# hahnyuan/PTQ4ViT

Hardware: AMD Instinct MI355X
Metric: calibration throughput (wrapped modules calibrated per second), ViT-B/224 W8A8, 32 calibration images (higher is better)
Workload: dtype int8

## Files before the change

### include/ptq4vit_hip.h

```cpp
#ifndef PTQ4VIT_HIP_H
#define PTQ4VIT_HIP_H

#include <stddef.h>
#include <stdint.h>

#ifdef __cplusplus
extern "C" {
#endif

#define P4V_VERSION 140

enum p4v_metric {
    P4V_METRIC_L1_NORM = 0,
    P4V_METRIC_L2_NORM = 1,
    P4V_METRIC_LINEAR_WEIGHTED_L2 = 2,
    P4V_METRIC_SQUARE_WEIGHTED_L2 = 3,
    P4V_METRIC_HESSIAN = 4,
    P4V_METRIC_COSINE = 5
};

enum p4v_status {
    P4V_OK = 0,
    P4V_ERR_INVALID = -1,
    P4V_ERR_UNSUPPORTED = -2,
    P4V_ERR_WORKSPACE = -3,
    P4V_ERR_HIP = -4
};

int p4v_version(void);
const char* p4v_last_error(void);

typedef struct p4v_linear_desc {
    int32_t batch;
    int32_t tokens;
    int32_t in_features;
    int32_t out_features;
    int32_t n_V, n_H, n_a;
    int32_t w_bit, a_bit;
    int32_t metric;
    int32_t eq_n;
    int32_t search_round;
    int32_t twin_postgelu;
    int32_t init_layerwise;
    int32_t has_bias;
    int32_t reserved;
} p4v_linear_desc;

size_t p4v_linear_workspace_bytes(const p4v_linear_desc* desc);

int p4v_linear_calibrate(const p4v_linear_desc* desc, const float* d_weight, const float* d_bias,
                         const float* d_x, const float* d_out, const float* d_grad, const float* d_mult,
                         float* d_w_interval, float* d_a_interval, float* d_scores, int32_t* d_best,
                         void* d_workspace, size_t workspace_bytes, void* stream);

typedef struct p4v_matmul_desc {
    int32_t batch, heads;
    int32_t M, K, N;
    int64_t a_stride[4];
    int64_t b_stride[4];
    int32_t A_bit, B_bit;
    int32_t metric;
    int32_t eq_n;
    int32_t search_round;
    int32_t sos;
    int32_t init_layerwise;
    int32_t reserved;
} p4v_matmul_desc;

size_t p4v_matmul_workspace_bytes(const p4v_matmul_desc* desc);

int p4v_matmul_calibrate(const p4v_matmul_desc* desc, const float* d_A, const float* d_B, const float* d_out,
                         const float* d_grad, const float* d_mult, float* d_A_interval, float* d_B_interval,
                         float* d_split, float* d_scores, int32_t* d_best, void* d_workspace,
                         size_t workspace_bytes, void* stream);

typedef struct p4v_conv_desc {
    int32_t batch, in_channels, height, width;
    int32_t out_channels, kernel_h, kernel_w;
    int32_t stride_h, stride_w, pad_h, pad_w, dil_h, dil_w;
    int32_t w_bit, a_bit;
    int32_t metric;
    int32_t eq_n;
    int32_t search_round;
    int32_t channelwise;
    int32_t init_layerwise;
    int32_t has_bias;
    int32_t reserved;
} p4v_conv_desc;

size_t p4v_conv_workspace_bytes(const p4v_conv_desc* desc);

int p4v_conv_calibrate(const p4v_conv_desc* desc, const float* d_weight, const float* d_bias, const float* d_x,
                       const float* d_out, const float* d_grad, const float* d_mult, float* d_w_interval,
                       float* d_a_interval, float* d_scores, int32_t* d_best, void* d_workspace,
                       size_t workspace_bytes, void* stream);

enum p4v_job_kind { P4V_JOB_LINEAR = 0, P4V_JOB_MATMUL = 1, P4V_JOB_CONV = 2 };
typedef struct p4v_group_job {
    int32_t kind;
    int32_t status;
    const void* desc;
    const float* in[5];
    const float* mult;
    float* out[3];
    void* workspace;
    size_t workspace_bytes;
} p4v_group_job;
int p4v_calibrate_group(p4v_group_job* jobs, int32_t n_jobs, void* stream, void* inputs_ready_event);

int p4v_launch_counters(int64_t* out4, int reset);


int p4v_amax_init_linear(const p4v_linear_desc* desc, const float* d_weight, const float* d_x, float* d_w_interval,
                         float* d_a_interval, void* d_workspace, size_t workspace_bytes, void* stream);

int p4v_linear_search_w(const p4v_linear_desc* desc, const float* d_weight, const float* d_bias, const float* d_x,
                        const float* d_out, const float* d_grad, const float* d_w_cands, float* d_w_interval,
                        const float* d_a_interval, float* d_scores, int32_t* d_best, void* d_workspace,
                        size_t workspace_bytes, void* stream);

int p4v_linear_search_a(const p4v_linear_desc* desc, const float* d_weight, const float* d_bias, const float* d_x,
                        const float* d_out, const float* d_grad, const float* d_a_cands, const float* d_w_interval,
                        float* d_a_interval, float* d_scores, int32_t* d_best, void* d_workspace, size_t workspace_bytes,
                        void* stream);

int p4v_amax_init_matmul(const p4v_matmul_desc* desc, const float* d_A, const float* d_B, float* d_A_interval,
                         float* d_B_interval, void* d_workspace, size_t workspace_bytes, void* stream);

int p4v_matmul_search_A(const p4v_matmul_desc* desc, const float* d_A, const float* d_B, const float* d_out,
                        const float* d_grad, const float* d_A_cands, float* d_A_interval, const float* d_B_interval,
                        float* d_scores, int32_t* d_best, void* d_workspace, size_t workspace_bytes, void* stream);

int p4v_sos_search_split(const p4v_matmul_desc* desc, const float* d_A, const float* d_B, const float* d_out,
                         const float* d_grad, float* d_split, float* d_A_interval, float* d_scores, int32_t* d_best,
                         void* d_workspace, size_t workspace_bytes, void* stream);

int p4v_matmul_search_B(const p4v_matmul_desc* desc, const float* d_A, const float* d_B, const float* d_out,
                        const float* d_grad, const float* d_B_cands, const float* d_A_interval, const float* d_split,
                        float* d_B_interval, float* d_scores, int32_t* d_best, void* d_workspace, size_t workspace_bytes,
                        void* stream);

int p4v_amax_init_conv(const p4v_conv_desc* desc, const float* d_weight, const float* d_x, float* d_w_interval,
                       float* d_a_interval, void* d_workspace, size_t workspace_bytes, void* stream);

int p4v_conv_search_w_channelwise(const p4v_conv_desc* desc, const float* d_weight, const float* d_bias, const float* d_x,
                                  const float* d_out, const float* d_grad, const float* d_w_cands, float* d_w_interval,
                                  const float* d_a_interval, float* d_scores, int32_t* d_best, void* d_workspace,
                                  size_t workspace_bytes, void* stream);

int p4v_conv_search_w_layerwise(const p4v_conv_desc* desc, const float* d_weight, const float* d_bias, const float* d_x,
                                const float* d_out, const float* d_grad, const float* d_w_cands, float* d_w_interval,
                                const float* d_a_interval, float* d_scores, int32_t* d_best, void* d_workspace,
                                size_t workspace_bytes, void* stream);

int p4v_conv_search_a(const p4v_conv_desc* desc, const float* d_weight, const float* d_bias, const float* d_x,
                      const float* d_out, const float* d_grad, const float* d_a_cands, const float* d_w_interval,
                      float* d_a_interval, float* d_scores, int32_t* d_best, void* d_workspace, size_t workspace_bytes,
                      void* stream);

int p4v_score_argmax_gather(const float* d_scores, int32_t eq_n, int32_t n_blocks, const float* d_cands,
                            float* d_interval, int32_t* d_best, void* stream);


int p4v_quantize_i8(const float* d_x, int64_t rows, int64_t cols, int64_t cols_padded, const float* d_scales,
                    int64_t rows_per_scale, int32_t lo, int32_t hi, int8_t* d_q, void* stream);

enum p4v_plane_mode { P4V_PLANE_SYM = 1, P4V_PLANE_SOS_HI = 2, P4V_PLANE_SOS_LO = 3, P4V_PLANE_TWIN = 4 };
typedef struct p4v_plane_desc {
    int64_t rows, cols, cols_padded;
    int64_t rows_per_scale;
    int32_t mode, lo, hi, qmax;
    float const_scale;
    int32_t reserved;
} p4v_plane_desc;
int p4v_pack_plane_i8(const p4v_plane_desc* desc, const float* d_x, const float* d_scales, int8_t* d_q, void* stream);

int p4v_fake_quant(const float* d_x, int64_t rows, int64_t cols, const float* d_scales, int64_t rows_per_scale,
                   int32_t lo, int32_t hi, float* d_y, void* stream);

enum p4v_export_mode { P4V_EXPORT_SYM_I8 = 0, P4V_EXPORT_SYM_F32 = 1, P4V_EXPORT_GELU_U8 = 2, P4V_EXPORT_SOS_U8 = 3 };
typedef struct p4v_export_desc {
    int32_t dims[4];
    int64_t src_stride[4];
    int64_t scale1_stride[4]; int32_t scale1_div[4];
    int64_t scale2_stride[4]; int32_t scale2_div[4];
    float scale2_const;
    int32_t mode, lo1, hi1, lo2, hi2, qmax;
    int32_t reserved;
} p4v_export_desc;
int p4v_export_quantize(const p4v_export_desc* desc, const float* d_src, const float* d_scale1, const float* d_scale2,
                        void* d_dst, void* stream);

int p4v_linear_quant_forward(const p4v_linear_desc* desc, const float* d_weight, const float* d_bias, const float* d_x,
                             const float* d_w_interval, const float* d_a_interval, float* d_out, void* d_workspace,
                             size_t workspace_bytes, void* stream);

int p4v_matmul_quant_forward(const p4v_matmul_desc* desc, const float* d_A, const float* d_B, const float* d_A_interval,
                             const float* d_B_interval, const float* d_split, float* d_out, void* d_workspace,
                             size_t workspace_bytes, void* stream);

int p4v_multi_copy(const int64_t* d_table, int32_t n, int64_t index, int64_t max_bytes, void* stream);

typedef struct p4v_kernel_stats {
    double sweep_i8_ms;
    int64_t sweep_i8_launches;
    double sweep_i8_macs;
    double sweep_f32_ms;
    int64_t sweep_f32_launches;
    double sweep_f32_macs;
    double sweep_i8_alg_macs;
    double sweep_f32_alg_macs;
    double sweep6_ms;
    int64_t sweep6_launches;
    double sweep6_macs;
    double sweep6_alg_macs;
    int64_t memo_hits;
    int64_t memo_misses;
    double sweep7_ms;
    int64_t sweep7_launches;
    double sweep7_macs;
    double sweep7_alg_macs;
    double sweep7_twin_ms;
    int64_t sweep7_twin_launches;
    double event_overhead_ms;
} p4v_kernel_stats;

typedef struct p4v_launch_record {
    int32_t kind;
    int32_t stage;
    int32_t grid_x, grid_z;
    double ms;
    double ops;
    double alg_ops;
    double alg_bytes;
} p4v_launch_record;
int p4v_stats_launches(p4v_launch_record* out, int64_t capacity, int64_t* count);

int p4v_stats_enable(int enable);
int p4v_stats_reset(void);
int p4v_stats_get(p4v_kernel_stats* out);

int p4v_prune_counters(int64_t* out4, int reset);


#ifdef __cplusplus
}
#endif
#endif
```

### include/ptq4vit_hip_debug.h

```cpp
#ifndef PTQ4VIT_HIP_DEBUG_H
#define PTQ4VIT_HIP_DEBUG_H

#include <stdint.h>

#ifdef __cplusplus
extern "C" {
#endif

int p4v_debug_set_variant(int variant, int force_generic);
int p4v_debug_set_tuning(int key, int value);
int p4v_debug_topk_rows(const float* d_mass, int segs, int n, int k, int32_t* d_idx, void* stream);
int p4v_debug_pack_dual(const float* d_x, long rows, long cols, long cols_padded, int sos, int lo, int hi, int qmax,
                        const float* d_scale, float const_scale, int8_t* d_q1, int8_t* d_q2, void* stream);
int p4v_debug_pack_cands(const float* d_x, long rows, long cols, long rows_padded, long cols_padded, int layout, int lo, int hi,
                         const float* d_scales, int n_cands, const int* d_crange, const unsigned char* d_done, int live_max,
                         int general, int8_t* d_q, void* stream);
int p4v_debug_prep_epi6(const float* d_o, const float* d_wt, const float* d_bias, long o_ss, long o_ts, int sr, int tr,
                        int bias_on_t, int wt_mode, int transposed, float* d_e, void* stream);

#ifdef __cplusplus
}
#endif
#endif
```

### ptq4vit_amd/_lib.py

```python
import ctypes as C
import os

_HERE = os.path.dirname(os.path.abspath(__file__))
LIB_PATH = os.environ.get("P4V_LIB") or os.path.join(_HERE, "csrc", "libptq4vit_hip.so")

METRICS = {
    "L1_norm": 0,
    "L2_norm": 1,
    "linear_weighted_L2_norm": 2,
    "square_weighted_L2_norm": 3,
    "hessian": 4,
    "cosine": 5,
}


class LinearDesc(C.Structure):
    _fields_ = [(n, C.c_int32) for n in (
        "batch", "tokens", "in_features", "out_features", "n_V", "n_H", "n_a", "w_bit", "a_bit", "metric",
        "eq_n", "search_round", "twin_postgelu", "init_layerwise", "has_bias", "reserved")]


class MatMulDesc(C.Structure):
    _fields_ = ([(n, C.c_int32) for n in ("batch", "heads", "M", "K", "N")] + [("_pad0", C.c_int32)] +
                [("a_stride", C.c_int64 * 4), ("b_stride", C.c_int64 * 4)] +
                [(n, C.c_int32) for n in ("A_bit", "B_bit", "metric", "eq_n", "search_round", "sos",
                                          "init_layerwise", "reserved")])


class ConvDesc(C.Structure):
    _fields_ = [(n, C.c_int32) for n in (
        "batch", "in_channels", "height", "width", "out_channels", "kernel_h", "kernel_w", "stride_h", "stride_w",
        "pad_h", "pad_w", "dil_h", "dil_w", "w_bit", "a_bit", "metric", "eq_n", "search_round", "channelwise",
        "init_layerwise", "has_bias", "reserved")]


class KernelStats(C.Structure):
    _fields_ = [("sweep_i8_ms", C.c_double), ("sweep_i8_launches", C.c_int64), ("sweep_i8_macs", C.c_double),
                ("sweep_f32_ms", C.c_double), ("sweep_f32_launches", C.c_int64), ("sweep_f32_macs", C.c_double),
                ("sweep_i8_alg_macs", C.c_double), ("sweep_f32_alg_macs", C.c_double),
                ("sweep6_ms", C.c_double), ("sweep6_launches", C.c_int64), ("sweep6_macs", C.c_double), ("sweep6_alg_macs", C.c_double),
                ("memo_hits", C.c_int64), ("memo_misses", C.c_int64),
                ("sweep7_ms", C.c_double), ("sweep7_launches", C.c_int64), ("sweep7_macs", C.c_double), ("sweep7_alg_macs", C.c_double),
                ("sweep7_twin_ms", C.c_double), ("sweep7_twin_launches", C.c_int64), ("event_overhead_ms", C.c_double)]


class LaunchRecord(C.Structure):
    _fields_ = [("kind", C.c_int32), ("stage", C.c_int32), ("grid_x", C.c_int32), ("grid_z", C.c_int32),
                ("ms", C.c_double), ("ops", C.c_double), ("alg_ops", C.c_double), ("alg_bytes", C.c_double)]


LAUNCH_KINDS = {0: "k_sweep<int8>", 1: "k_sweep<float>", 2: "k_sweep6", 3: "k_sweep7", 4: "k_sweep7 (twin)", 5: "k_sweep4/5", 6: "k_sweep9",
                7: "k_sweep8", 8: "k_sweep2g", 9: "k_sweep2", 11: "k_sos_split", 12: "k_bound", 13: "k_slice_b", 14: "k_slice_a"}
LAUNCH_STAGES = {0: "full", 1: "A", 2: "B1", 3: "B2", 4: "A2"}


class PlaneDesc(C.Structure):
    _fields_ = [("rows", C.c_int64), ("cols", C.c_int64), ("cols_padded", C.c_int64), ("rows_per_scale", C.c_int64),
                ("mode", C.c_int32), ("lo", C.c_int32), ("hi", C.c_int32), ("qmax", C.c_int32),
                ("const_scale", C.c_float), ("reserved", C.c_int32)]


class ExportDesc(C.Structure):
    _fields_ = [("dims", C.c_int32 * 4), ("src_stride", C.c_int64 * 4),
                ("scale1_stride", C.c_int64 * 4), ("scale1_div", C.c_int32 * 4),
                ("scale2_stride", C.c_int64 * 4), ("scale2_div", C.c_int32 * 4),
                ("scale2_const", C.c_float),
                ("mode", C.c_int32), ("lo1", C.c_int32), ("hi1", C.c_int32), ("lo2", C.c_int32), ("hi2", C.c_int32),
                ("qmax", C.c_int32), ("reserved", C.c_int32)]


class GroupJob(C.Structure):
    _fields_ = [("kind", C.c_int32), ("status", C.c_int32), ("desc", C.c_void_p), ("inp", C.c_void_p * 5), ("mult", C.c_void_p),
                ("out", C.c_void_p * 3), ("workspace", C.c_void_p), ("workspace_bytes", C.c_size_t)]


JOB_LINEAR, JOB_MATMUL, JOB_CONV = 0, 1, 2
PLANE_SYM, PLANE_SOS_HI, PLANE_SOS_LO, PLANE_TWIN = 1, 2, 3, 4
EXPORT_SYM_I8, EXPORT_SYM_F32, EXPORT_GELU_U8, EXPORT_SOS_U8 = 0, 1, 2, 3


EXPORTS = [
    "p4v_version", "p4v_last_error",
    "p4v_linear_workspace_bytes", "p4v_linear_calibrate",
    "p4v_matmul_workspace_bytes", "p4v_matmul_calibrate",
    "p4v_conv_workspace_bytes", "p4v_conv_calibrate",
    "p4v_calibrate_group", "p4v_launch_counters",
    "p4v_linear_quant_forward", "p4v_matmul_quant_forward",
    "p4v_amax_init_linear", "p4v_linear_search_w", "p4v_linear_search_a",
    "p4v_amax_init_matmul", "p4v_matmul_search_A", "p4v_sos_search_split", "p4v_matmul_search_B",
    "p4v_amax_init_conv", "p4v_conv_search_w_channelwise", "p4v_conv_search_w_layerwise", "p4v_conv_search_a",
    "p4v_score_argmax_gather",
    "p4v_quantize_i8", "p4v_pack_plane_i8", "p4v_fake_quant", "p4v_export_quantize", "p4v_multi_copy",
    "p4v_stats_enable", "p4v_stats_reset", "p4v_stats_get", "p4v_stats_launches", "p4v_prune_counters",
    "p4v_debug_set_variant", "p4v_debug_set_tuning", "p4v_debug_topk_rows", "p4v_debug_pack_dual", "p4v_debug_prep_epi6",
    "p4v_debug_pack_cands",
]

_lib = None


def load():
    global _lib
    if _lib is not None:
        return _lib
    if not os.path.exists(LIB_PATH):
        raise RuntimeError(
            f"ptq4vit_amd: HIP extension {LIB_PATH} is missing -- build it with "
            "`python -c 'import __graft_entry__ as g; g.build()'` (hipcc --offload-arch=gfx950). "
            "There is no CPU fallback for the calibration path.")
    import torch
    lib = C.CDLL(LIB_PATH)
    vp, fp, ip = C.c_void_p, C.c_void_p, C.c_void_p
    lib.p4v_version.restype = C.c_int
    lib.p4v_last_error.restype = C.c_char_p
    lib.p4v_linear_workspace_bytes.restype = C.c_size_t
    lib.p4v_linear_workspace_bytes.argtypes = [C.POINTER(LinearDesc)]
    lib.p4v_linear_calibrate.restype = C.c_int
    lib.p4v_linear_calibrate.argtypes = [C.POINTER(LinearDesc), fp, fp, fp, fp, fp, fp, fp, fp, fp, ip, vp, C.c_size_t, vp]
    lib.p4v_matmul_workspace_bytes.restype = C.c_size_t
    lib.p4v_matmul_workspace_bytes.argtypes = [C.POINTER(MatMulDesc)]
    lib.p4v_matmul_calibrate.restype = C.c_int
    lib.p4v_matmul_calibrate.argtypes = [C.POINTER(MatMulDesc), fp, fp, fp, fp, fp, fp, fp, fp, fp, ip, vp, C.c_size_t, vp]
    lib.p4v_conv_workspace_bytes.restype = C.c_size_t
    lib.p4v_conv_workspace_bytes.argtypes = [C.POINTER(ConvDesc)]
    lib.p4v_conv_calibrate.restype = C.c_int
    lib.p4v_conv_calibrate.argtypes = [C.POINTER(ConvDesc), fp, fp, fp, fp, fp, fp, fp, fp, fp, ip, vp, C.c_size_t, vp]
    lib.p4v_linear_quant_forward.restype = C.c_int
    lib.p4v_linear_quant_forward.argtypes = [C.POINTER(LinearDesc), fp, fp, fp, fp, fp, fp, vp, C.c_size_t, vp]
    lib.p4v_matmul_quant_forward.restype = C.c_int
    lib.p4v_matmul_quant_forward.argtypes = [C.POINTER(MatMulDesc), fp, fp, fp, fp, fp, fp, vp, C.c_size_t, vp]
    LD, MD, CD = C.POINTER(LinearDesc), C.POINTER(MatMulDesc), C.POINTER(ConvDesc)
    tail = [vp, C.c_size_t, vp]
    for name, args in (
            ("p4v_amax_init_linear", [LD] + [fp] * 4),
            ("p4v_linear_search_w", [LD] + [fp] * 9 + [ip]),
            ("p4v_linear_search_a", [LD] + [fp] * 9 + [ip]),
            ("p4v_amax_init_matmul", [MD] + [fp] * 4),
            ("p4v_matmul_search_A", [MD] + [fp] * 8 + [ip]),
            ("p4v_sos_search_split", [MD] + [fp] * 7 + [ip]),
            ("p4v_matmul_search_B", [MD] + [fp] * 9 + [ip]),
            ("p4v_amax_init_conv", [CD] + [fp] * 4),
            ("p4v_conv_search_w_channelwise", [CD] + [fp] * 9 + [ip]),
            ("p4v_conv_search_w_layerwise", [CD] + [fp] * 9 + [ip]),
            ("p4v_conv_search_a", [CD] + [fp] * 9 + [ip])):
        fn = getattr(lib, name)
        fn.restype = C.c_int
        fn.argtypes = args + tail
    lib.p4v_score_argmax_gather.restype = C.c_int
    lib.p4v_score_argmax_gather.argtypes = [fp, C.c_int32, C.c_int32, fp, fp, ip, vp]
    lib.p4v_quantize_i8.restype = C.c_int
    lib.p4v_quantize_i8.argtypes = [fp, C.c_int64, C.c_int64, C.c_int64, fp, C.c_int64, C.c_int32, C.c_int32, vp, vp]
    lib.p4v_fake_quant.restype = C.c_int
    lib.p4v_fake_quant.argtypes = [fp, C.c_int64, C.c_int64, fp, C.c_int64, C.c_int32, C.c_int32, fp, vp]
    lib.p4v_pack_plane_i8.restype = C.c_int
    lib.p4v_pack_plane_i8.argtypes = [C.POINTER(PlaneDesc), fp, fp, vp, vp]
    lib.p4v_export_quantize.restype = C.c_int
    lib.p4v_export_quantize.argtypes = [C.POINTER(ExportDesc), fp, fp, fp, vp, vp]
    lib.p4v_multi_copy.restype = C.c_int
    lib.p4v_multi_copy.argtypes = [vp, C.c_int32, C.c_int64, C.c_int64, vp]
    lib.p4v_debug_topk_rows.restype = C.c_int
    lib.p4v_debug_topk_rows.argtypes = [vp, C.c_int, C.c_int, C.c_int, vp, vp]
    lib.p4v_debug_pack_dual.restype = C.c_int
    lib.p4v_debug_pack_dual.argtypes = [fp, C.c_long, C.c_long, C.c_long, C.c_int, C.c_int, C.c_int, C.c_int, fp, C.c_float, vp, vp, vp]
    lib.p4v_debug_pack_cands.restype = C.c_int
    lib.p4v_debug_pack_cands.argtypes = [fp, C.c_long, C.c_long, C.c_long, C.c_long, C.c_int, C.c_int, C.c_int, fp, C.c_int, vp, vp,
                                         C.c_int, C.c_int, vp, vp]
    lib.p4v_debug_prep_epi6.restype = C.c_int
    lib.p4v_debug_prep_epi6.argtypes = [fp, fp, fp, C.c_long, C.c_long, C.c_int, C.c_int, C.c_int, C.c_int, C.c_int, fp, vp]
    lib.p4v_debug_set_variant.restype = C.c_int
    lib.p4v_debug_set_variant.argtypes = [C.c_int, C.c_int]
    lib.p4v_debug_set_tuning.restype = C.c_int
    lib.p4v_debug_set_tuning.argtypes = [C.c_int, C.c_int]
    lib.p4v_stats_enable.restype = C.c_int
    lib.p4v_stats_enable.argtypes = [C.c_int]
    lib.p4v_stats_reset.restype = C.c_int
    lib.p4v_stats_get.restype = C.c_int
    lib.p4v_stats_get.argtypes = [C.POINTER(KernelStats)]
    lib.p4v_stats_launches.restype = C.c_int
    lib.p4v_stats_launches.argtypes = [C.POINTER(LaunchRecord), C.c_int64, C.POINTER(C.c_int64)]
    lib.p4v_prune_counters.restype = C.c_int
    lib.p4v_prune_counters.argtypes = [C.POINTER(C.c_int64), C.c_int]
    lib.p4v_launch_counters.restype = C.c_int
    lib.p4v_launch_counters.argtypes = [C.POINTER(C.c_int64), C.c_int]
    lib.p4v_calibrate_group.restype = C.c_int
    lib.p4v_calibrate_group.argtypes = [C.POINTER(GroupJob), C.c_int32, vp, vp]
    _lib = lib
    return lib


def check(rc, what):
    if rc != 0:
        msg = load().p4v_last_error().decode("utf-8", "replace")
        if rc == -2:
            raise NotImplementedError(f"{what}: {msg}")
        raise RuntimeError(f"{what} failed (code {rc}): {msg}")


def source_hash():
    import hashlib
    root = os.path.dirname(os.path.abspath(__file__))
    h = hashlib.sha256()
    for rel in ("csrc/p4v_kernels.h", "csrc/p4v_api.hip", "../include/ptq4vit_hip.h"):
        with open(os.path.join(root, rel), "rb") as f:
            h.update(f.read())
    return h.hexdigest()[:16]
```

### ptq4vit_amd/csrc/p4v_api.hip

```cpp
#include <hip/hip_runtime.h>

#include <algorithm>
#include <atomic>
#include <climits>
#include <cstdarg>
#include <cstdio>
#include <condition_variable>
#include <cstring>
#include <deque>
#include <functional>
#include <thread>
#include <mutex>
#include <string>
#include <unordered_map>
#include <type_traits>
#include <vector>

#include "../../include/ptq4vit_hip.h"
#include "../../include/ptq4vit_hip_debug.h"
#include "p4v_kernels.h"

using namespace p4v;

namespace {
// ... 24 lines not shown
inline long rup(long x, long m) { return (x + m - 1) / m * m; }
inline int cdiv(long a, long b) { return (int)((a + b - 1) / b); }

struct Arena {
    char* base;
    size_t cap, off, peak;
    size_t top;
    bool dry;
    Arena(void* b, size_t c) : base((char*)b), cap(c & ~(size_t)255), off(0), peak(0), top(0), dry(b == nullptr) {}
    template <typename T> T* get(size_t n) {
        off = (size_t)rup((long)off, 256);
        T* p = dry ? nullptr : (T*)(base + off);
        off += n * sizeof(T);
        if (off + top > peak) peak = off + top;
        return p;
    }
    char* get_top(size_t bytes) {
        top += (size_t)rup((long)bytes, 256);
        if (off + top > peak) peak = off + top;
        return (dry || top > cap) ? nullptr : base + cap - top;
    }
    bool ok() const { return dry || off + top <= cap; }
};

struct StatRec { hipEvent_t a, b; int kind; double macs, alg; int stage, gx, gz; double ms, bytes; };
thread_local double g_alg_bytes = 0;
thread_local double g_alg_macs_cand = 0;
thread_local double g_exec_frac = 1.0;
thread_local bool g_stat_on = false;
thread_local std::vector<StatRec> g_stat_recs;
thread_local std::vector<StatRec> g_stat_done;
thread_local int g_stage = 0;
thread_local p4v_kernel_stats g_stats = {};
thread_local long g_memo_hits = 0, g_memo_misses = 0;
std::atomic<long long> g_prune_cnt[4];
constexpr int VARIANT_KEPT = 1 | 2 | 4 | 2048 | 32768 | 65536 | 131072 | 524288 | 1048576 | 2097152 | 4194304 | 8388608 | 134217728;
std::atomic<int> g_variant_word{0};
#define g_variant (g_variant_word.load(std::memory_order_relaxed) & 0x3fffffff)
#define g_force_v1 ((g_variant_word.load(std::memory_order_relaxed) >> 30) & 1)
std::atomic<int> g_tune[16];
enum { TUNE_CG6 = 0, TUNE_CG2 = 1, TUNE_CG2G = 2, TUNE_CG7 = 3, TUNE_PRINT = 4, TUNE_ORDER7 = 5, TUNE_P6 = 6, TUNE_PLANE_GIB = 7, TUNE_EPI6W = 8,
       TUNE_LOOSE_PCT = 9, TUNE_SLICE_DIV = 10, TUNE_SLICE_SMALL = 11, TUNE_B1_PATH = 12, TUNE_TIER2 = 13, TUNE_TIER2_DIV = 14, TUNE_LOOSE_ROWS = 15 };
inline bool tune_b1_removed(int v) { return v == 1 || v == 2 || v == 3 || v == 5 || v == 6 || v == 8 || v == 10 || v == 12; }
inline int tune(int k) { return g_tune[k].load(std::memory_order_relaxed); }

struct Group;
struct Ctx {
    hipStream_t st;
    Arena ws;
    bool dry;
    Group* grp = nullptr;
    int slot = 0;
    int par = 1;
};

struct StatInfo { int kind; double macs, alg; int stage, gx, gz; double bytes; };
struct QOp;
struct KernelDesc {
    hipError_t (*one)(const QOp&, hipStream_t);
    hipError_t (*many)(const QOp* const*, int, hipStream_t);
    int cap;
};
constexpr int QOP_PARAM_BYTES = 480;
struct QOp {
    enum Type : int { KERNEL, FILL, D2H, H2D, COPY2D, WAIT };
    int type = KERNEL;
    const KernelDesc* kd = nullptr;
    dim3 grid, block;
    unsigned lds = 0;
    alignas(16) char params[QOP_PARAM_BYTES];
    void* dst = nullptr; const void* src = nullptr; size_t bytes = 0; int value = 0;
    size_t dpitch = 0, spitch = 0, width = 0, height = 0;
    std::vector<char> payload;
    bool timed = false;
    bool heavy = false;
    StatInfo si{};
};
inline hipError_t lds_attr(const void* fn, unsigned lds, std::atomic<bool>& done) {
    if (lds <= 48 * 1024 || done.load(std::memory_order_acquire)) return hipSuccess;
    const hipError_t e = hipFuncSetAttribute(fn, hipFuncAttributeMaxDynamicSharedMemorySize, 160 * 1024);
    if (e == hipSuccess) done.store(true, std::memory_order_release);
    return e;
}
template <typename P, void (*K1)(P), void (*KG)(GroupArgs<P>)> struct Kern {
    static_assert(sizeof(P) <= QOP_PARAM_BYTES, "kernel parameter block larger than a queued operation holds");
    static hipError_t one(const QOp& op, hipStream_t st) {
        static std::atomic<bool> attr{false};
        if (hipError_t e = lds_attr((const void*)K1, op.lds, attr); e != hipSuccess) return e;
        P p;
        std::memcpy(&p, op.params, sizeof(P));
        void* args[] = {&p};
        return hipLaunchKernel((const void*)K1, op.grid, op.block, args, op.lds, st);
    }
    static hipError_t many(const QOp* const* ops, int n, hipStream_t st) {
        static std::atomic<bool> attr{false};
        GroupArgs<P> a;
        unsigned off = 0, lds = 0;
        a.n = n;
        for (int m = 0; m < n; ++m) {
            const QOp& op = *ops[m];
            a.off[m] = off; a.gx[m] = op.grid.x; a.gy[m] = op.grid.y; a.gz[m] = op.grid.z;
            std::memcpy(&a.p[m], op.params, sizeof(P));
            off += (unsigned)rup((long)op.grid.x * op.grid.y * op.grid.z, 8);
            lds = std::max(lds, op.lds);
        }
        a.off[n] = off;
        if (hipError_t e = lds_attr((const void*)KG, lds, attr); e != hipSuccess) return e;
// ... 1059 lines not shown
        const bool cosp = ps.cos6 || ps.cos7;
        const int cos6_FS = !cosp ? 0 : ps.cos_ZV == 1 ? cos6_slabs : ps.sb_div / cos_slab;
        FinishCosParams fp{part, p_cs, cosp ? (long)cos6_FS * cos6_Sp * 3 : p_zs, cosp ? cos6_Sp : Np, cosp ? cos6_FS : MT,
                           ps.cos_ZB, ps.cos_ZV, cosp ? ps.Mrows : ps.Ncols, ps.eq_n,
                           ps.cos_j_mode, std::max(1, ps.cos_j_div), ps.nj, ps.norm, scores};
        CHK(launch_finish_cos(c, fp));
    }
    if (!ps.no_select) {
        SelectParams sl{scores, ps.eq_n, ps.nj, ps.cands, ps.cand_cs, ps.cand_js, ps.cand_off, ps.interval, ps.out_js,
                        ps.out_off, ps.aux_out, ps.aux_div, ps.scores_out, ps.scores_out_ld, ps.best_out};
        CHK(launch_select(c, sl));
    }
    c.ws.off = mark;
    return 0;
}

struct SliceGeo {
    bool lin; int segs, seg_rows, k , Ncols, K;
    const float* O; const float* G; int wt_mode; long o_ms;
    const float* row_src; long s_r, s_k; int zdiv; long s_z2, s_z;
    bool conv; PackParams conv_pk;
    int k_cap;
};
int slice_alloc(Ctx& c, SliceCache* sc, const SliceGeo& g, bool keep, bool bump) {
    if (sc->assigned) {
        if (sc->k != g.k_cap) return fail(P4V_ERR_INVALID, "slice cache reused with another geometry");
        return 0;
    }
    if (!keep && !bump) return 0;
    const long zrows = (long)g.segs * g.seg_rows, out_elems = (long)g.segs * g.k_cap * g.Ncols, row_elems = (long)g.segs * g.k_cap * g.K;
    if (keep) {
        sc->idx = reinterpret_cast<int*>(c.ws.get_top((size_t)g.segs * g.k_cap * sizeof(int)));
        sc->mass = reinterpret_cast<float*>(c.ws.get_top((size_t)zrows * sizeof(float)));
        sc->Os = reinterpret_cast<float*>(c.ws.get_top((size_t)out_elems * sizeof(float)));
        sc->Gs = reinterpret_cast<float*>(c.ws.get_top((size_t)out_elems * sizeof(float)));
        sc->Rs = reinterpret_cast<float*>(c.ws.get_top((size_t)row_elems * sizeof(float)));
        sc->frac = reinterpret_cast<float*>(c.ws.get_top(256));
        sc->assigned = true;
    } else {
        sc->idx = c.ws.get<int>((size_t)g.segs * g.k_cap);
        sc->mass = c.ws.get<float>((size_t)zrows);
        sc->Os = c.ws.get<float>((size_t)out_elems);
        sc->Gs = c.ws.get<float>((size_t)out_elems);
        sc->Rs = c.ws.get<float>((size_t)row_elems);
    }
    sc->k = g.k_cap;
    return 0;
}
int slice_fill(Ctx& c, SliceCache* sc, const SliceGeo& g, bool host_sync_ok) {
    const long zrows = (long)g.segs * g.seg_rows;
    const void* wsrc = g.G ? (const void*)g.G : (const void*)g.O;
    const bool new_idx = sc->idx_src != wsrc || sc->idx_wt != g.wt_mode || (g.wt_mode != 1 && sc->o_src != g.O);
    if (new_idx) {
        CHK(enqueue(c, KERN(RowMassParams, k_row_mass), dim3((unsigned)cdiv(zrows, 4)), dim3(256), 0, RowMassParams{g.G ? g.G : g.O, g.O, zrows, (long)g.Ncols, g.wt_mode, sc->mass}));
        CHK(enqueue(c, KERN(TopkParams, k_topk_rows), dim3(g.segs), dim3(1024), 0, TopkParams{sc->mass, g.seg_rows, g.k, sc->idx}));
        sc->idx_src = wsrc; sc->idx_wt = g.wt_mode;
        sc->o_src = sc->g_src = sc->r_src = nullptr;
        if (sc->frac && host_sync_ok && !(g_variant & 8388608)) {
            float f = 1.0f;
            int* hm = host_mirror(c);
            CHK(enqueue(c, KERN(MassFracParams, k_mass_fraction), dim3(1), dim3(1024), 0,
                        MassFracParams{sc->mass, zrows, sc->idx, g.segs, g.seg_rows, g.k, sc->frac, hm ? reinterpret_cast<float*>(hm + 4) : nullptr}));
            if (!hm) CHK(q_d2h(c, &f, sc->frac, sizeof f));
            CHK(q_sync(c));
            if (hm) f = *reinterpret_cast<volatile float*>(hm + 4);
            if (tune(TUNE_PRINT) > 0) fprintf(stderr, "[p4v] slice holds %.4f of the metric weight (%d x %d of %d rows)\n", f, g.segs, g.k, g.seg_rows);
            sc->frac_host = f;
            if (g.k < g.k_cap && !(f >= 0.97f)) {
                SliceGeo g2 = g;
                g2.k = g.k_cap;
                sc->idx_src = nullptr;
                return slice_fill(c, sc, g2, host_sync_ok);
            }
            const bool big_pass = zrows >= (tune(TUNE_LOOSE_ROWS) > 0 ? (long)tune(TUNE_LOOSE_ROWS) : 65536L);
            if (!(f >= (tune(TUNE_LOOSE_PCT) > 0 ? 0.01f * tune(TUNE_LOOSE_PCT) : big_pass ? 0.05f : 0.5f))) { sc->loose = true; return 0; }
        }
        sc->k_eff = g.k;
    }
    const int rows = g.segs * g.k;
    int gather_rc = 0;
    auto gather = [&](const float* src, long s0, long s3, int d3, float* dst, int seg, int zdiv, long sz2, long sz) {
        GatherParams gp{src, s0, 0, 0, s3, 1, 1, d3, sc->idx, rows, dst, seg, zdiv, sz2, sz};
        const long total = (long)rows * d3;
        if (const int r_ = enqueue(c, KERN(GatherParams, k_gather), dim3((unsigned)std::min<long>(cdiv(total, 256), 256L * 16)), dim3(256), 0, gp)) gather_rc = r_;
    };
    const int seg = g.lin ? 0 : g.k;
    const long o_seg = (long)g.seg_rows * g.Ncols;
    if (sc->o_src != g.O) { gather(g.O, g.o_ms, 1, g.Ncols, sc->Os, seg, 1, o_seg, 0); sc->o_src = g.O; }
    if (g.G && sc->g_src != g.G) { gather(g.G, g.o_ms, 1, g.Ncols, sc->Gs, seg, 1, o_seg, 0); sc->g_src = g.G; }
    if (sc->r_src != g.row_src) {
        if (g.conv) {
            const long total = (long)rows * g.K;
            CHK(enqueue(c, KERN(GatherIm2colParams, k_gather_im2col), dim3((unsigned)std::min<long>(cdiv(total, 256), 256L * 16)), dim3(256), 0, GatherIm2colParams{g.conv_pk, sc->idx, rows, sc->Rs}));
        } else if (g.lin) gather(g.row_src, g.s_r, 1, g.K, sc->Rs, 0, 1, 0, 0);
        else gather(g.row_src, g.s_r, g.s_k, g.K, sc->Rs, g.k, g.zdiv, g.s_z2, g.s_z);
        sc->r_src = g.row_src;
        sc->aplane.valid = false;
    }
    return gather_rc;
}

bool prune_ok(const Pass& ps) {
    if (!ps.prunable || !(ps.i8 || ps.prunable_f32) || ps.epi == EPI_COS || ps.store_out || ps.scores_out || ps.best_out || ps.crange || ps.no_select) return false;
    if ((g_variant & 4194304) || ps.eq_n < 32 || ps.nj < 1 || ps.nj > 4096) return false;
    return true;
}
int launch_pass_select(Ctx& c, const Pass& ps, const float* scores) {
    SelectParams sl{scores, ps.eq_n, ps.nj, ps.cands, ps.cand_cs, ps.cand_js, ps.cand_off, ps.interval, ps.out_js,
                    ps.out_off, ps.aux_out, ps.aux_div, ps.scores_out, ps.scores_out_ld, ps.best_out};
    return launch_select(c, sl);
}

#define PRUNE_COUNT(i) do { if (!c.dry) g_prune_cnt[i].fetch_add(1, std::memory_order_relaxed); } while (0)
constexpr int PRUNE_FP32_CHAIN = 128 + 6;
inline float prune_margin() { return std::max(1e-4f, 4.0f * 2.0f * (float)PRUNE_FP32_CHAIN * 5.9604645e-8f); }
// ... 477 lines not shown
    bool full() const { return mask == ST_ALL; }
    bool searches() const { return (mask & (ST_S1 | ST_S2)) != 0; }
};

PackParams pack2d(const float* src, long rows, long cols, long ld) {
    PackParams p{};
    p.src = src; p.s_z = 0; p.s_r = ld; p.s_k = 1; p.Z = 1; p.R = (int)rows; p.K = (int)cols;
    p.mode = PACK_SYM; p.nblk_r = 1; p.nblk_k = 1;
    return p;
}

int linear_impl(const p4v_linear_desc* d, const float* W, const float* bias, const float* X, const float* O,
                const float* G, const float* mult, float* w_iv, float* a_iv, float* scores_out, int32_t* best_out,
                Ctx& c, float* fwd_out = nullptr, const Stage& sg = Stage{}) {
    const int M = d->batch * d->tokens, K = d->in_features, N = d->out_features;
    const int nV = d->n_V, nH = d->n_H, nA = d->n_a;
    if (M <= 0 || K <= 0 || N <= 0 || nV <= 0 || nH <= 0 || nA <= 0 || d->eq_n <= 0)
        return fail(P4V_ERR_INVALID, "linear: non-positive dimension");
    if (N % nV || K % nH || K % nA) return fail(P4V_ERR_UNSUPPORTED, "linear: n_V/n_H/n_a must divide the layer (reference ignores remainders, linear.py:118)");
    if (d->w_bit > 8 || d->a_bit > 8 || d->w_bit < 2 || d->a_bit < 2) return fail(P4V_ERR_UNSUPPORTED, "linear: bit widths 2..8 supported");
    const int crb_rows = N / nV, crb_cols = K / nH, crb_acts = K / nA;
    const int wq = 1 << (d->w_bit - 1), aq = 1 << (d->a_bit - 1);
    const float a_neg = (float)(0.16997124254703522 / aq);
    int epi, wt_mode;
    metric_epi(d->metric, &epi, &wt_mode);
    const bool cosm = epi == EPI_COS;
    if (wt_mode == 1 && !G && !fwd_out && sg.searches()) return fail(P4V_ERR_INVALID, "linear: hessian metric needs raw_grad (linear.py:418)");
    const bool general = (nH > 1 || nA > 1 || (d->reserved & 1) || (cosm && d->twin_postgelu && !fwd_out));
    const bool i8 = !general;
    const bool twin = d->twin_postgelu && i8;
    if (cosm && !fwd_out && (nH > 1 || nA > 1)) return fail(P4V_ERR_UNSUPPORTED, "linear: cosine with n_H>1 / n_a>1 is not implemented on the GPU");
    const int ncand = d->eq_n + 1;

    cvt_bias(c);
    unsigned* enc_w = c.ws.get<unsigned>((size_t)nV * nH);
    unsigned* enc_a = c.ws.get<unsigned>((size_t)nA);
    float* w_cands_ws = c.ws.get<float>((size_t)ncand * nV * nH);
    float* a_cands_ws = c.ws.get<float>((size_t)ncand * nA);
    const float* w_cands = (sg.mask & ST_INIT) ? w_cands_ws : sg.cands1;
    const float* a_cands = (sg.mask & ST_INIT) ? a_cands_ws : sg.cands2;
    float* Ufold = twin ? c.ws.get<float>((size_t)M * N) : nullptr;
    float* w_mix = c.ws.get<float>((size_t)ncand * nV * nH);
    float* a_mix = c.ws.get<float>((size_t)ncand * nA);
    if (!c.ws.ok()) return fail(P4V_ERR_WORKSPACE, "workspace too small");
    if (!fwd_out && (sg.mask & ST_INIT)) {
        const long stw[4] = {0, 0, K, 1};
        CHK(launch_absmax(c, W, stw, 1, 1, N, K, nV, nH, crb_rows, crb_cols, 0, enc_w));
        CHK(launch_interval(c, enc_w, nV * nH, (float)(wq - 0.5), d->init_layerwise, w_iv));
        if (sg.searches()) CHK(launch_cands(c, mult, w_iv, ncand, nV * nH, w_cands_ws));
    }
    auto init_activation_side = [&]() -> int {
        if (!fwd_out && (sg.mask & ST_INIT)) {
            const long stw[4] = {0, 0, K, 1};
            CHK(launch_absmax(c, X, stw, 1, 1, M, K, 1, nA, M, crb_acts, d->twin_postgelu ? 1 : 0, enc_a));
            CHK(launch_interval(c, enc_a, nA, (float)(aq - 0.5), d->init_layerwise, a_iv));
            if (sg.searches()) CHK(launch_cands(c, mult, a_iv, ncand, nA, a_cands_ws));
        }
        return 0;
    };
    if (fwd_out || !sg.full()) {
        CHK(q_wait_inputs(c));
        CHK(init_activation_side());
    }
    if (!fwd_out && !sg.searches()) return 0;

    auto x_operand = [&](bool expanded, const float* scales, int sc_cs) {
        Operand op{};
        op.present = true; op.expanded = expanded;
        op.pk = pack2d(X, M, K, K);
        op.pk.scales = scales; op.pk.sc_cs = sc_cs;
        op.pk.lo = -aq; op.pk.hi = aq - 1;
        if (nA > 1) { op.pk.blk_mode = 1; op.pk.blk_div = INT_MAX; op.pk.nblk_r = 1; op.pk.nblk_k = nA; op.pk.blk_div2 = crb_acts; }
        if (d->twin_postgelu) {
            if (i8) { op.pk.lo = 0; }
            else { op.pk.mode = PACK_TWIN_SIM; op.pk.lo = -aq; op.pk.neg_scale = a_neg; }
        }
        return op;
    };
    auto xneg_operand = [&]() {
        Operand op{};
        op.present = true; op.expanded = false;
        op.pk = pack2d(X, M, K, K);
        op.pk.scales = nullptr; op.pk.neg_scale = a_neg; op.pk.lo = -aq; op.pk.hi = 0;
        return op;
    };
    auto w_operand = [&](bool expanded, const float* scales, int sc_cs, bool by_vblock) {
        Operand op{};
        op.present = true; op.expanded = expanded;
        if (by_vblock) {
            op.pk = pack2d(W, crb_rows, K, K);
            op.pk.s_z = (long)crb_rows * K;
            op.pk.blk_mode = 2; op.pk.blk_div = nV;
            if (nH > 1) return op;
        } else {
            op.pk = pack2d(W, N, K, K);
            op.pk.blk_mode = 1; op.pk.blk_div = crb_rows; op.pk.nblk_r = nV; op.pk.nblk_k = nH;
            op.pk.blk_div2 = nH > 1 ? crb_cols : 0;
        }
        op.pk.scales = scales; op.pk.sc_cs = sc_cs;
        op.pk.lo = -wq; op.pk.hi = wq - 1;
        return op;
    };

    if (fwd_out) {
        Pass fp{};
        fp.i8 = i8; fp.twin = twin; fp.epi = EPI_FWD; fp.wt_mode = 0; fp.eq_n = 1; fp.K = K;
        fp.Z = 1; fp.Mrows = M; fp.Ncols = N;
        fp.row = x_operand(false, a_iv, 0);
// ... 154 lines not shown
                    slice2.o_src = nullptr;
                }
                if (cos6 || cos7) cos6_pass(ps, 0);
            } else {
                ps.Z = nV; ps.Mrows = crb_rows; ps.Ncols = M;
                ps.row = w_operand(false, w_iv, 0, true);
                ps.col = x_operand(true, ac, nA);
                ps.col_zs_shared = 1;
                ps.use_s1 = i8; ps.s_cs = nV; ps.sb_mode = 2; ps.sb_div = nV;
                ps.s1 = ScaleParams{a_cands, 1, 0, 0.f, w_iv, 0, 1, 0.f, 0, 0, nullptr};
                ps.bias = bias; ps.bias_axis = 1; ps.bias_zs = crb_rows;
                ps.O = O; ps.o_zs = crb_rows; ps.o_ms = 1; ps.o_ns = N; ps.o_inner = INT_MAX;
                ps.cos_ZB = 1; ps.cos_ZV = nV; ps.cos_j_mode = 0;
                ps.norm = 1.0 / (double)d->tokens;
            }
            CHK(run_pass_pruned(c, ps));
        }
        if (memo_a_on && !skip_a) { CHK(read_dev(c, a_iv, nA, val)); memo_a.entries.push_back({key, val}); g_memo_misses++; host_a = val; host_a_ok = true; }
        else if (!skip_a) host_a_ok = false;
    }
    return 0;
}

int matmul_impl(const p4v_matmul_desc* d, const float* A, const float* B, const float* O, const float* G,
                const float* mult, float* A_iv, float* B_iv, float* split, float* scores_out, int32_t* best_out, Ctx& c,
                float* fwd_out = nullptr, const Stage& sg = Stage{}) {
    const int H = d->heads, Z = d->batch * d->heads, M = d->M, K = d->K, N = d->N;
    if (Z <= 0 || M <= 0 || K <= 0 || N <= 0 || d->eq_n <= 0) return fail(P4V_ERR_INVALID, "matmul: non-positive dimension");
    if (d->A_bit > 8 || d->B_bit > 8) return fail(P4V_ERR_UNSUPPORTED, "matmul: bit widths <= 8 supported");
    const int Aq = 1 << (d->A_bit - 1), Bq = 1 << (d->B_bit - 1);
    int epi, wt_mode;
    metric_epi(d->metric, &epi, &wt_mode);
    const bool cosm = epi == EPI_COS;
    if (wt_mode == 1 && !G && !fwd_out && sg.searches()) return fail(P4V_ERR_INVALID, "matmul: hessian metric needs raw_grad");
    if (d->sos && !split) return fail(P4V_ERR_INVALID, "matmul: sos needs d_split");
    cvt_bias(c);
    CHK(q_wait_inputs(c));
    const int ncand = d->eq_n + 1;
    const int NSPLIT = 20;

    unsigned* enc_A = c.ws.get<unsigned>(H);
    unsigned* enc_B = c.ws.get<unsigned>(H);
    float* A_cands_ws = c.ws.get<float>((size_t)ncand * H);
    float* B_cands_ws = c.ws.get<float>((size_t)ncand * H);
    const float* A_cands = (sg.mask & ST_INIT) ? A_cands_ws : sg.cands1;
    const float* B_cands = (sg.mask & ST_INIT) ? B_cands_ws : sg.cands2;
    float* split_cands = c.ws.get<float>(NSPLIT);
    float* A_headwise = c.ws.get<float>(H);
    if (!c.ws.ok()) return fail(P4V_ERR_WORKSPACE, "workspace too small");
    if (!fwd_out && (sg.mask & ST_INIT)) {
        const long sa[4] = {d->a_stride[0], d->a_stride[1], d->a_stride[2], d->a_stride[3]};
        const long sb[4] = {d->b_stride[0], d->b_stride[1], d->b_stride[2], d->b_stride[3]};
        float* a_dst = d->sos ? A_headwise : A_iv;
        CHK(launch_absmax(c, A, sa, d->batch, H, M, K, 1, 1, M, K, 0, enc_A));
        CHK(launch_interval(c, enc_A, H, (float)(Aq - 0.5), d->init_layerwise, a_dst));
        CHK(launch_absmax(c, B, sb, d->batch, H, K, N, 1, 1, K, N, 0, enc_B));
        CHK(launch_interval(c, enc_B, H, (float)(Bq - 0.5), d->init_layerwise, B_iv));
        if (sg.searches()) {
            if (!d->sos) CHK(launch_cands(c, mult, A_iv, ncand, H, A_cands_ws));
            CHK(launch_cands(c, mult, B_iv, ncand, H, B_cands_ws));
        }
    }
    if (!fwd_out && !sg.searches()) return 0;
    if (!fwd_out && (sg.mask & ST_S1)) {
        if (d->sos && !c.dry) {
            float sc[NSPLIT];
            for (int i = 0; i < NSPLIT; ++i) sc[i] = (float)std::ldexp(1.0, -i);
            CHK(q_h2d(c, split_cands, sc, sizeof sc));
            if (!c.grp) CHK(q_sync(c));
        }
    }
    auto A_operand = [&](bool expanded, const float* scales, int sc_cs, int mode) {
        Operand op{};
        op.present = true; op.expanded = expanded;
        op.pk = PackParams{};
        op.pk.src = A; op.pk.s_z = d->a_stride[1]; op.pk.s_r = d->a_stride[2]; op.pk.s_k = d->a_stride[3];
        op.pk.s_z2 = d->a_stride[0]; op.pk.zdiv = H;
        op.pk.Z = Z; op.pk.R = M; op.pk.K = K; op.pk.nblk_r = 1; op.pk.nblk_k = 1;
        op.pk.mode = mode; op.pk.scales = scales; op.pk.sc_cs = sc_cs;
        op.pk.blk_mode = (mode == PACK_SYM) ? 2 : 0; op.pk.blk_div = H;
        op.pk.lo = -Aq; op.pk.hi = Aq - 1; op.pk.qm1 = (float)(Aq - 1);
        return op;
    };
    auto B_operand = [&](bool expanded, const float* scales, int sc_cs, int mode) {
        Operand op{};
        op.present = true; op.expanded = expanded;
        op.pk = PackParams{};
        op.pk.src = B; op.pk.s_z = d->b_stride[1]; op.pk.s_r = d->b_stride[3]; op.pk.s_k = d->b_stride[2];
        op.pk.s_z2 = d->b_stride[0]; op.pk.zdiv = H;
        op.pk.Z = Z; op.pk.R = N; op.pk.K = K; op.pk.nblk_r = 1; op.pk.nblk_k = 1;
        op.pk.mode = mode; op.pk.scales = scales; op.pk.sc_cs = sc_cs;
        op.pk.blk_mode = (mode == PACK_SYM) ? 2 : 0; op.pk.blk_div = H;
        op.pk.lo = -Bq; op.pk.hi = Bq - 1;
        return op;
    };
    auto common = [&](Pass& ps) {
        ps.Z = Z; ps.K = K;
        ps.O = O; ps.G = G; ps.wt_mode = wt_mode; ps.epi = epi;
        ps.o_inner = INT_MAX;
        if (!cosm) { ps.Mrows = M; ps.Ncols = N; ps.o_zs = (long)M * N; ps.o_ms = N; ps.o_ns = 1; }
        else { ps.Mrows = N; ps.Ncols = M; ps.o_zs = (long)M * N; ps.o_ms = 1; ps.o_ns = N; ps.G = nullptr;
               ps.cos_ZB = Z; ps.cos_ZV = 1; }
    };

    if (fwd_out) {
        Pass fp{};
        fp.Z = Z; fp.K = K; fp.Mrows = M; fp.Ncols = N;
        fp.i8 = true; fp.twin = d->sos; fp.epi = EPI_FWD; fp.wt_mode = 0; fp.eq_n = 1;
        fp.row = d->sos ? A_operand(false, split, 0, PACK_SOS_HI) : A_operand(false, A_iv, 0, PACK_SYM);
        if (d->sos) fp.row2 = A_operand(false, split, 0, PACK_SOS_LO);
// ... 104 lines not shown
                ps.s1 = ScaleParams{nullptr, 0, 0, 1.0f / (float)(Aq - 1), B_cands, H, 1, 0.f, 0, 0, nullptr};
                ps.s2 = ScaleParams{A_iv, 0, 0, 0.f, B_cands, H, 1, 0.f, 0, 0, nullptr};
            }
            ps.j_mode = 2; ps.j_div = H; ps.nj = H; ps.cos_j_mode = 2; ps.cos_j_div = H;
            ps.norm = cosm ? 1.0 / (double)M : 1.0 / ((double)M * N);
            ps.cands = B_cands; ps.cand_cs = H; ps.cand_js = 1; ps.interval = B_iv; ps.out_js = 1;
            ps.cache = keep_planes ? &plane_B : nullptr;
            ps.scores_out = so_B; ps.scores_out_ld = H;
            ps.best_out = bo_B;
            ps.prunable = !cosm && ps.i8 && !(d->reserved & 8); ps.scache = &slice; ps.host_sync_ok = memo_on;
            CHK(run_pass_pruned(c, ps));
            if (memo_on) { CHK(read_dev(c, B_iv, H, val)); memo_B.entries.push_back({key, val}); g_memo_misses++; }
        }
    }
    return 0;
}

int conv_impl(const p4v_conv_desc* d, const float* W, const float* bias, const float* X, const float* O, const float* G,
              const float* mult, float* w_iv, float* a_iv, float* scores_out, int32_t* best_out, Ctx& c,
              const Stage& sg = Stage{}) {
    const int b = d->batch, ic = d->in_channels, H = d->height, Wd = d->width, oc = d->out_channels;
    const int kh = d->kernel_h, kw = d->kernel_w;
    const int fh = (H + 2 * d->pad_h - d->dil_h * (kh - 1) - 1) / d->stride_h + 1;
    const int fw = (Wd + 2 * d->pad_w - d->dil_w * (kw - 1) - 1) / d->stride_w + 1;
    if (b <= 0 || ic <= 0 || oc <= 0 || fh <= 0 || fw <= 0 || d->eq_n <= 0) return fail(P4V_ERR_INVALID, "conv: bad geometry");
    if (d->w_bit > 8) return fail(P4V_ERR_UNSUPPORTED, "conv: w_bit <= 8 supported");
    const int L = fh * fw, K = ic * kh * kw, M = b * L;
    const int wq = 1 << (d->w_bit - 1);
    const bool aquant = d->a_bit < 32;
    const int aq = aquant ? (1 << (d->a_bit - 1)) : 0;
    if (aquant && !d->channelwise) return fail(P4V_ERR_UNSUPPORTED, "conv: the layer-wise class cannot search activations (reference conv.py:420 raises IndexError); use a_bit=32");
    cvt_bias(c);
    CHK(q_wait_inputs(c));
    int epi, wt_mode;
    metric_epi(d->metric, &epi, &wt_mode);
    const bool cosm = epi == EPI_COS;
    if (wt_mode == 1 && !G && sg.searches()) return fail(P4V_ERR_INVALID, "conv: hessian metric needs raw_grad");
    if (cosm && aquant) return fail(P4V_ERR_UNSUPPORTED, "conv: cosine does not support the activation search (reference conv.py:505-506)");
    const int nw = d->channelwise ? oc : 1;
    const int ncand = d->eq_n + 1;

    unsigned* enc_w = c.ws.get<unsigned>(nw);
    unsigned* enc_a = c.ws.get<unsigned>(1);
    float* w_cands_ws = c.ws.get<float>((size_t)ncand * nw);
    float* a_cands_ws = c.ws.get<float>(ncand);
    const float* w_cands = (sg.mask & ST_INIT) ? w_cands_ws : sg.cands1;
    const float* a_cands = (sg.mask & ST_INIT) ? a_cands_ws : sg.cands2;
    if (!c.ws.ok()) return fail(P4V_ERR_WORKSPACE, "workspace too small");
    if (sg.mask & ST_INIT) {
        const long stw[4] = {0, 0, K, 1};
        CHK(launch_absmax(c, W, stw, 1, 1, oc, K, nw, 1, d->channelwise ? 1 : oc, K, 0, enc_w));
        CHK(launch_interval(c, enc_w, nw, (float)(wq - 0.5), d->init_layerwise, w_iv));
        const long stx[4] = {0, 0, (long)ic * H * Wd, 1};
        CHK(launch_absmax(c, X, stx, 1, 1, b, ic * H * Wd, 1, 1, b, ic * H * Wd, 0, enc_a));
        CHK(launch_interval(c, enc_a, 1, aquant ? (float)(aq - 0.5) : (float)(std::ldexp(1.0, d->a_bit - 1) - 0.5), 0, a_iv));
        if (sg.searches()) {
            CHK(launch_cands(c, mult, w_iv, ncand, nw, w_cands_ws));
            CHK(launch_cands(c, mult, a_iv, ncand, 1, a_cands_ws));
        }
    }
    if (!sg.searches()) return 0;
    const bool prunable = !cosm && sg.full() && !scores_out && !best_out && !(d->reserved & 8) && d->eq_n >= 32;
    float* Ot = prunable ? c.ws.get<float>((size_t)M * oc) : nullptr;
    float* Gt = (prunable && G) ? c.ws.get<float>((size_t)M * oc) : nullptr;
    if (!c.ws.ok()) return fail(P4V_ERR_WORKSPACE, "workspace too small");
    if (prunable && !c.dry) {
        const dim3 grid(cdiv(L, 32), cdiv(oc, 32), b);
        CHK(enqueue(c, KERN(NchwRowsParams, k_nchw_to_rows), grid, dim3(256), 0, NchwRowsParams{O, oc, L, Ot}));
        if (G) CHK(enqueue(c, KERN(NchwRowsParams, k_nchw_to_rows), grid, dim3(256), 0, NchwRowsParams{G, oc, L, Gt}));
    }
    auto x_operand = [&](bool expanded, const float* scales, int sc_cs, bool per_image) {
        Operand op{};
        op.present = true; op.expanded = expanded;
        op.pk = PackParams{};
        op.pk.src = X; op.pk.conv = 1; op.pk.ic = ic; op.pk.H = H; op.pk.W = Wd; op.pk.kh = kh; op.pk.kw = kw;
        op.pk.sh = d->stride_h; op.pk.sw = d->stride_w; op.pk.ph = d->pad_h; op.pk.pw = d->pad_w; op.pk.dh = d->dil_h; op.pk.dw = d->dil_w;
        op.pk.fw = fw; op.pk.L = L;
        op.pk.Z = per_image ? b : 1; op.pk.s_z = per_image ? (long)ic * H * Wd : 0;
        op.pk.R = per_image ? L : M; op.pk.K = K; op.pk.nblk_r = 1; op.pk.nblk_k = 1;
        op.pk.mode = aquant ? PACK_SYM : PACK_RAW; op.pk.scales = aquant ? scales : nullptr; op.pk.sc_cs = sc_cs;
        op.pk.lo = -aq; op.pk.hi = aq - 1;
        return op;
    };
    auto w_operand = [&](bool expanded, const float* scales, int sc_cs) {
        Operand op{};
        op.present = true; op.expanded = expanded;
        op.pk = pack2d(W, oc, K, K);
        op.pk.scales = scales; op.pk.sc_cs = sc_cs;
        op.pk.blk_mode = d->channelwise ? 1 : 0; op.pk.blk_div = 1; op.pk.nblk_r = nw; op.pk.nblk_k = 1;
        op.pk.lo = -wq; op.pk.hi = wq - 1;
        return op;
    };
    auto setup = [&](Pass& ps, bool w_search) {
        ps.i8 = false; ps.twin = false; ps.epi = epi; ps.wt_mode = wt_mode; ps.eq_n = d->eq_n; ps.K = K;
        ps.use_s1 = false; ps.s_cs = 1; ps.sb_mode = 0;
        ps.O = O; ps.G = G; ps.bias = bias;
        Operand xo = x_operand(!w_search, w_search ? a_iv : a_cands, w_search ? 0 : 1, cosm && d->channelwise);
        Operand wo = w_operand(w_search, w_search ? w_cands : w_iv, w_search ? nw : 0);
        if (!cosm) {
            ps.Z = 1; ps.Mrows = M; ps.Ncols = oc; ps.row = xo; ps.col = wo;
            ps.o_inner = L; ps.o_bs = (long)oc * L; ps.o_ms = 1; ps.o_ns = L; ps.bias_axis = 0;
            if (prunable) { ps.O = Ot; ps.G = G ? Gt : nullptr; ps.o_inner = INT_MAX; ps.o_bs = 0; ps.o_ms = oc; ps.o_ns = 1; }
        } else if (d->channelwise) {
            ps.Z = b; ps.Mrows = L; ps.Ncols = oc; ps.row = xo; ps.col = wo; ps.col_zs_shared = 1;
            ps.o_zs = (long)oc * L; ps.o_inner = INT_MAX; ps.o_ms = 1; ps.o_ns = L; ps.bias_axis = 0; ps.G = nullptr;
            ps.cos_ZB = b; ps.cos_ZV = 1;
        } else {
            ps.Z = 1; ps.Mrows = oc; ps.Ncols = M; ps.row = wo; ps.col = xo;
// ... 157 lines not shown
    return linear_impl(desc, d_weight, desc->has_bias ? d_bias : nullptr, d_x, nullptr, nullptr, nullptr,
                       const_cast<float*>(d_w_interval), const_cast<float*>(d_a_interval), nullptr, nullptr, c, d_out);
}

int p4v_matmul_quant_forward(const p4v_matmul_desc* desc, const float* d_A, const float* d_B, const float* d_A_interval,
                             const float* d_B_interval, const float* d_split, float* d_out, void* d_workspace,
                             size_t workspace_bytes, void* stream) {
    if (!desc || !d_A || !d_B || !d_A_interval || !d_B_interval || !d_out || !d_workspace)
        return fail(P4V_ERR_INVALID, "p4v_matmul_quant_forward: null pointer");
    if (desc->sos && !d_split) return fail(P4V_ERR_INVALID, "p4v_matmul_quant_forward: sos needs d_split");
    Ctx c{(hipStream_t)stream, Arena(d_workspace, workspace_bytes), false};
    return matmul_impl(desc, d_A, d_B, nullptr, nullptr, nullptr, const_cast<float*>(d_A_interval),
                       const_cast<float*>(d_B_interval), const_cast<float*>(d_split), nullptr, nullptr, c, d_out);
}

size_t p4v_matmul_workspace_bytes(const p4v_matmul_desc* desc) {
    if (!desc) return 0;
    Ctx c{nullptr, Arena(nullptr, 0), true};
    float dummy = 0;
    float* fwd = (desc->reserved & 4) ? (float*)16 : nullptr;
    if (matmul_impl(desc, nullptr, nullptr, nullptr, (const float*)1, nullptr, nullptr, nullptr, &dummy, nullptr, nullptr, c, fwd) != 0) return 0;
    return c.ws.peak + 4096;
}

int p4v_matmul_calibrate(const p4v_matmul_desc* desc, const float* d_A, const float* d_B, const float* d_out,
                         const float* d_grad, const float* d_mult, float* d_A_interval, float* d_B_interval, float* d_split,
                         float* d_scores, int32_t* d_best, void* d_workspace, size_t workspace_bytes, void* stream) {
    if (!desc || !d_A || !d_B || !d_out || !d_mult || !d_A_interval || !d_B_interval || !d_workspace)
        return fail(P4V_ERR_INVALID, "matmul: null pointer");
    Ctx c{(hipStream_t)stream, Arena(d_workspace, workspace_bytes), false};
    return matmul_impl(desc, d_A, d_B, d_out, d_grad, d_mult, d_A_interval, d_B_interval, d_split, d_scores, d_best, c);
}

size_t p4v_conv_workspace_bytes(const p4v_conv_desc* desc) {
    if (!desc) return 0;
    Ctx c{nullptr, Arena(nullptr, 0), true};
    if (conv_impl(desc, nullptr, nullptr, nullptr, nullptr, (const float*)1, nullptr, nullptr, nullptr, nullptr, nullptr, c) != 0) return 0;
    return c.ws.peak + 4096;
}

int p4v_conv_calibrate(const p4v_conv_desc* desc, const float* d_weight, const float* d_bias, const float* d_x,
                       const float* d_out, const float* d_grad, const float* d_mult, float* d_w_interval, float* d_a_interval,
                       float* d_scores, int32_t* d_best, void* d_workspace, size_t workspace_bytes, void* stream) {
    if (!desc || !d_weight || !d_x || !d_out || !d_mult || !d_w_interval || !d_a_interval || !d_workspace)
        return fail(P4V_ERR_INVALID, "conv: null pointer");
    if (desc->has_bias && !d_bias) return fail(P4V_ERR_INVALID, "conv: has_bias set but d_bias is NULL");
    Ctx c{(hipStream_t)stream, Arena(d_workspace, workspace_bytes), false};
    return conv_impl(desc, d_weight, desc->has_bias ? d_bias : nullptr, d_x, d_out, d_grad, d_mult, d_w_interval, d_a_interval,
                     d_scores, d_best, c);
}


int p4v_calibrate_group(p4v_group_job* jobs, int32_t n_jobs, void* stream, void* inputs_ready_event) {
    if (n_jobs < 0 || (n_jobs > 0 && !jobs)) return fail(P4V_ERR_INVALID, "p4v_calibrate_group: bad job list");
    if (n_jobs == 0) return 0;
    for (int i = 0; i < n_jobs; ++i) {
        jobs[i].status = 0;
        if (!jobs[i].desc || group_desc_bytes(jobs[i].kind) == 0) return fail(P4V_ERR_INVALID, "p4v_calibrate_group: member %d has no descriptor / an unknown kind", i);
    }
    int dev = 0;
    HIPCHK(hipGetDevice(&dev));
    cvt_probe((hipStream_t)stream);
    Group g;
    g.st = (hipStream_t)stream; g.n = n_jobs;
    g.q.resize(n_jobs); g.state.assign(n_jobs, 0); g.mirrors.resize(n_jobs);
    for (int i = 0; i < n_jobs; ++i) g.mirrors[i] = group_mirror(g.st, dev, i);
    g.stat_on = g_stat_on;
    g.stat_recs = g_stat_on ? &g_stat_recs : nullptr;
    g.inputs_ready = (hipEvent_t)inputs_ready_event;
    g_launch_cnt[3].fetch_add(1, std::memory_order_relaxed);
    std::vector<std::string> errs(n_jobs);
    std::atomic<long> memo_hits{0}, memo_misses{0};
    std::mutex dmu;
    std::condition_variable dcv;
    int left = n_jobs;
    for (int i = 0; i < n_jobs; ++i) {
        int par = 0;
        for (int k = 0; k < n_jobs; ++k)
            par += jobs[k].kind == jobs[i].kind && std::memcmp(jobs[k].desc, jobs[i].desc, group_desc_bytes(jobs[i].kind)) == 0;
        worker_pool().run([&, i, par] {
            (void)hipSetDevice(dev);
            g_stat_on = g.stat_on; g_stage = 0; g_exec_frac = 1.0; g_memo_hits = 0; g_memo_misses = 0; g_err.clear();
            Ctx c{g.st, Arena(jobs[i].workspace, jobs[i].workspace_bytes), false, &g, i, par};
            const int r = run_group_member(jobs[i], c);
            jobs[i].status = r;
            if (r) errs[i] = g_err;
            memo_hits += g_memo_hits; memo_misses += g_memo_misses;
            g_stat_on = false;
            g.finish(i);
            std::lock_guard<std::mutex> lk(dmu);
            if (--left == 0) dcv.notify_all();
        });
    }
    {
        std::unique_lock<std::mutex> lk(dmu);
        dcv.wait(lk, [&] { return left == 0; });
    }
    g_memo_hits += memo_hits.load(); g_memo_misses += memo_misses.load();
    if (tune(TUNE_PRINT) > 0) fprintf(stderr, "[p4v] group of %d: %ld launches asked for, %ld issued in %ld rounds\n", n_jobs, g.n_ops, g.n_launches, g.n_rounds);
    if (g.status) { g_err = g.err; return g.status; }
    for (int i = 0; i < n_jobs; ++i)
        if (jobs[i].status) { g_err = errs[i]; return jobs[i].status; }
    return 0;
}

int p4v_launch_counters(int64_t* out4, int reset) {
    if (out4) for (int i = 0; i < 4; ++i) out4[i] = (int64_t)g_launch_cnt[i].load(std::memory_order_relaxed);
    if (reset) for (int i = 0; i < 4; ++i) g_launch_cnt[i].store(0, std::memory_order_relaxed);
    return 0;
}

int p4v_amax_init_linear(const p4v_linear_desc* desc, const float* d_weight, const float* d_x, float* d_w_interval,
                         float* d_a_interval, void* d_workspace, size_t workspace_bytes, void* stream) {
    if (!desc || !d_weight || !d_x || !d_w_interval || !d_a_interval || !d_workspace)
        return fail(P4V_ERR_INVALID, "p4v_amax_init_linear: null pointer");
    Ctx c{(hipStream_t)stream, Arena(d_workspace, workspace_bytes), false};
    return linear_impl(desc, d_weight, nullptr, d_x, nullptr, nullptr, nullptr, d_w_interval, d_a_interval, nullptr, nullptr, c,
                       nullptr, Stage{ST_INIT, nullptr, nullptr});
}

int p4v_linear_search_w(const p4v_linear_desc* desc, const float* d_weight, const float* d_bias, const float* d_x,
                        const float* d_out, const float* d_grad, const float* d_w_cands, float* d_w_interval,
                        const float* d_a_interval, float* d_scores, int32_t* d_best, void* d_workspace,
                        size_t workspace_bytes, void* stream) {
    if (!desc || !d_weight || !d_x || !d_out || !d_w_cands || !d_w_interval || !d_a_interval || !d_workspace)
        return fail(P4V_ERR_INVALID, "p4v_linear_search_w: null pointer");
    if (desc->has_bias && !d_bias) return fail(P4V_ERR_INVALID, "p4v_linear_search_w: has_bias set but d_bias is NULL");
    Ctx c{(hipStream_t)stream, Arena(d_workspace, workspace_bytes), false};
    return linear_impl(desc, d_weight, desc->has_bias ? d_bias : nullptr, d_x, d_out, d_grad, nullptr, d_w_interval,
                       const_cast<float*>(d_a_interval), d_scores, d_best, c, nullptr, Stage{ST_S1, d_w_cands, nullptr});
}

int p4v_linear_search_a(const p4v_linear_desc* desc, const float* d_weight, const float* d_bias, const float* d_x,
                        const float* d_out, const float* d_grad, const float* d_a_cands, const float* d_w_interval,
                        float* d_a_interval, float* d_scores, int32_t* d_best, void* d_workspace, size_t workspace_bytes,
                        void* stream) {
// ... 76 lines not shown
int p4v_conv_search_w_channelwise(const p4v_conv_desc* desc, const float* d_weight, const float* d_bias, const float* d_x,
                                  const float* d_out, const float* d_grad, const float* d_w_cands, float* d_w_interval,
                                  const float* d_a_interval, float* d_scores, int32_t* d_best, void* d_workspace,
                                  size_t workspace_bytes, void* stream) {
    return conv_search("p4v_conv_search_w_channelwise", 1, ST_S1, desc, d_weight, d_bias, d_x, d_out, d_grad, d_w_cands,
                       d_w_interval, const_cast<float*>(d_a_interval), d_scores, d_best, d_workspace, workspace_bytes, stream);
}

int p4v_conv_search_w_layerwise(const p4v_conv_desc* desc, const float* d_weight, const float* d_bias, const float* d_x,
                                const float* d_out, const float* d_grad, const float* d_w_cands, float* d_w_interval,
                                const float* d_a_interval, float* d_scores, int32_t* d_best, void* d_workspace,
                                size_t workspace_bytes, void* stream) {
    return conv_search("p4v_conv_search_w_layerwise", 0, ST_S1, desc, d_weight, d_bias, d_x, d_out, d_grad, d_w_cands,
                       d_w_interval, const_cast<float*>(d_a_interval), d_scores, d_best, d_workspace, workspace_bytes, stream);
}

int p4v_conv_search_a(const p4v_conv_desc* desc, const float* d_weight, const float* d_bias, const float* d_x,
                      const float* d_out, const float* d_grad, const float* d_a_cands, const float* d_w_interval,
                      float* d_a_interval, float* d_scores, int32_t* d_best, void* d_workspace, size_t workspace_bytes,
                      void* stream) {
    if (desc && desc->a_bit >= 32) return fail(P4V_ERR_INVALID, "p4v_conv_search_a: a_bit >= 32 leaves the input unquantised (conv.py:600)");
    return conv_search("p4v_conv_search_a", -1, ST_S2, desc, d_weight, d_bias, d_x, d_out, d_grad, d_a_cands,
                       const_cast<float*>(d_w_interval), d_a_interval, d_scores, d_best, d_workspace, workspace_bytes, stream);
}

int p4v_score_argmax_gather(const float* d_scores, int32_t eq_n, int32_t n_blocks, const float* d_cands, float* d_interval,
                            int32_t* d_best, void* stream) {
    if (!d_scores || !d_cands || !d_interval || eq_n <= 0 || n_blocks <= 0)
        return fail(P4V_ERR_INVALID, "p4v_score_argmax_gather: bad argument");
    Ctx c{(hipStream_t)stream, Arena(nullptr, 0), false};
    SelectParams sl{d_scores, eq_n, n_blocks, d_cands, n_blocks, 1, 0, d_interval, 1, 0, nullptr, 0.0f, nullptr, 0, d_best};
    return launch_select(c, sl);
}

int p4v_quantize_i8(const float* d_x, int64_t rows, int64_t cols, int64_t cols_padded, const float* d_scales,
                    int64_t rows_per_scale, int32_t lo, int32_t hi, int8_t* d_q, void* stream) {
    if (!d_x || !d_scales || !d_q || rows <= 0 || cols <= 0 || cols_padded % 64 || cols_padded < cols || rows_per_scale <= 0)
        return fail(P4V_ERR_INVALID, "quantize_i8: bad argument");
    Ctx c{(hipStream_t)stream, Arena(nullptr, 0), false};
    PackParams p = pack2d(d_x, rows, cols, cols);
    p.Rp = (int)rows; p.Kp = (int)cols_padded; p.dst = d_q; p.C = 1;
    p.scales = d_scales; p.sc_cs = 0; p.blk_mode = 1; p.blk_div = (int)rows_per_scale;
    p.nblk_r = cdiv(rows, rows_per_scale); p.nblk_k = 1; p.lo = lo; p.hi = hi;
    return launch_pack<int8_t>(c, p);
}

int p4v_fake_quant(const float* d_x, int64_t rows, int64_t cols, const float* d_scales, int64_t rows_per_scale,
                   int32_t lo, int32_t hi, float* d_y, void* stream) {
    if (!d_x || !d_scales || !d_y || rows <= 0 || cols <= 0 || rows_per_scale <= 0)
        return fail(P4V_ERR_INVALID, "fake_quant: bad argument");
    const long n = rows * cols;
    hipLaunchKernelGGL(k_fake_quant_rows, dim3((unsigned)std::min<long>(cdiv(n, 256), 65536)), dim3(256), 0,
                       (hipStream_t)stream, d_x, (long)rows, (long)cols, d_scales, (long)rows_per_scale, (float)lo, (float)hi, d_y);
    HIPCHK(hipGetLastError());
    return 0;
}

int p4v_multi_copy(const int64_t* d_table, int32_t n, int64_t index, int64_t max_bytes, void* stream) {
    if (!d_table || n <= 0 || index < 0 || max_bytes <= 0) return fail(P4V_ERR_INVALID, "p4v_multi_copy: bad argument");
    static_assert(sizeof(long) == sizeof(int64_t), "table entries are 64-bit");
    const unsigned gx = (unsigned)std::max<long>(1, std::min<long>(cdiv(max_bytes / 16, 256 * 8), 256));
    hipLaunchKernelGGL(k_multi_copy, dim3(gx, (unsigned)n), dim3(256), 0, (hipStream_t)stream, (const long*)d_table, (long)index);
    HIPCHK(hipGetLastError());
    return 0;
}

thread_local double g_evt_overhead_ms = 0.0;
int p4v_stats_enable(int enable) {
    g_stat_on = enable != 0;
    if (g_stat_on) {
        hipEvent_t a, b;
        HIPCHK(hipEventCreate(&a));
        HIPCHK(hipEventCreate(&b));
        double best = 1e9;
        for (int i = 0; i < 32; ++i) {
            HIPCHK(hipEventRecord(a, nullptr));
            HIPCHK(hipEventRecord(b, nullptr));
            HIPCHK(hipEventSynchronize(b));
            float ms = 0;
            HIPCHK(hipEventElapsedTime(&ms, a, b));
            best = std::min(best, (double)ms);
        }
        hipEventDestroy(a);
        hipEventDestroy(b);
        g_evt_overhead_ms = best < 1e8 ? best : 0.0;
    }
    return 0;
}

static int stats_drain() {
    for (auto& r : g_stat_recs) {
        HIPCHK(hipEventSynchronize(r.b));
        float ms = 0;
        HIPCHK(hipEventElapsedTime(&ms, r.a, r.b));
        ms = (float)std::max(0.0, (double)ms - g_evt_overhead_ms);
        if (r.kind == 0 || (r.kind >= 2 && r.kind <= 9) || (r.kind >= 12 && r.kind <= 14)) { g_stats.sweep_i8_ms += ms; g_stats.sweep_i8_launches++; g_stats.sweep_i8_macs += r.macs; g_stats.sweep_i8_alg_macs += r.alg; }
        if (r.kind == 2) { g_stats.sweep6_ms += ms; g_stats.sweep6_launches++; g_stats.sweep6_macs += r.macs; g_stats.sweep6_alg_macs += r.alg; }
        if (r.kind == 3 || r.kind == 4) { g_stats.sweep7_ms += ms; g_stats.sweep7_launches++; g_stats.sweep7_macs += r.macs; g_stats.sweep7_alg_macs += r.alg; }
        if (r.kind == 4) { g_stats.sweep7_twin_ms += ms; g_stats.sweep7_twin_launches++; }
        if (r.kind == 1 || r.kind == 11) { g_stats.sweep_f32_ms += ms; g_stats.sweep_f32_launches++; g_stats.sweep_f32_macs += r.macs; g_stats.sweep_f32_alg_macs += r.alg; }
        hipEventDestroy(r.a);
        hipEventDestroy(r.b);
        r.ms = ms;
        g_stat_done.push_back(r);
    }
    g_stat_recs.clear();
    return 0;
}

int p4v_stats_reset(void) {
    int r = stats_drain();
    g_stats = p4v_kernel_stats{};
    g_stat_done.clear();
    g_memo_hits = 0; g_memo_misses = 0;
    return r;
}

int p4v_stats_get(p4v_kernel_stats* out) {
    if (!out) return fail(P4V_ERR_INVALID, "stats_get: null");
    int r = stats_drain();
    g_stats.memo_hits = g_memo_hits; g_stats.memo_misses = g_memo_misses;
    g_stats.event_overhead_ms = g_evt_overhead_ms;
    *out = g_stats;
    return r;
}

int p4v_stats_launches(p4v_launch_record* out, int64_t capacity, int64_t* count) {
    int r = stats_drain();
    if (r) return r;
    if (count) *count = (int64_t)g_stat_done.size();
    if (out)
        for (int64_t i = 0; i < capacity && i < (int64_t)g_stat_done.size(); ++i) {
            const StatRec& s = g_stat_done[(size_t)i];
            out[i] = p4v_launch_record{s.kind, s.stage, s.gx, s.gz, (double)s.ms, 2.0 * s.macs, 2.0 * s.alg, s.bytes};
        }
    return 0;
}

int p4v_prune_counters(int64_t* out4, int reset) {
    if (out4) for (int i = 0; i < 4; ++i) out4[i] = (int64_t)g_prune_cnt[i].load(std::memory_order_relaxed);
    if (reset) for (int i = 0; i < 4; ++i) g_prune_cnt[i].store(0, std::memory_order_relaxed);
    return 0;
}

int p4v_debug_set_variant(int variant, int force_generic) {
    if (variant < 0 || variant >= (1 << 30)) return fail(P4V_ERR_INVALID, "p4v_debug_set_variant: bad variant word");
    if (variant & ~VARIANT_KEPT) return fail(P4V_ERR_INVALID, "p4v_debug_set_variant: bits 0x%x select removed paths", variant & ~VARIANT_KEPT);
    g_variant_word.store(variant | (force_generic ? (1 << 30) : 0), std::memory_order_relaxed);
    return 0;
}

int p4v_debug_set_tuning(int key, int value) {
    if (key < 0 || key >= 16) return fail(P4V_ERR_INVALID, "p4v_debug_set_tuning: unknown key %d", key);
    if (key == TUNE_B1_PATH && tune_b1_removed(value)) return fail(P4V_ERR_INVALID, "p4v_debug_set_tuning: 12 = %d selects a removed path", value);
    g_tune[key].store(value, std::memory_order_relaxed);
    return 0;
}

int p4v_debug_topk_rows(const float* d_mass, int segs, int n, int k, int32_t* d_idx, void* stream) {
    if (!d_mass || !d_idx || segs <= 0 || n <= 0 || k <= 0 || k > n) return fail(P4V_ERR_INVALID, "p4v_debug_topk_rows: bad argument");
    hipLaunchKernelGGL(k_topk_rows, dim3(segs), dim3(1024), 0, (hipStream_t)stream, TopkParams{d_mass, n, k, d_idx});
    HIPCHK(hipGetLastError());
    return 0;
}

int p4v_debug_pack_dual(const float* d_x, long rows, long cols, long cols_padded, int sos, int lo, int hi, int qmax,
                        const float* d_scale, float const_scale, int8_t* d_q1, int8_t* d_q2, void* stream) {
    if (!d_x || !d_scale || !d_q1 || !d_q2 || rows <= 0 || cols <= 0 || cols_padded % 64 || cols_padded < cols ||
        lo > 0 || hi < 0 || lo < -128 || hi > 127 || qmax < 2 || qmax > 128 || (!sos && !(const_scale > 0.0f)))
        return fail(P4V_ERR_INVALID, "p4v_debug_pack_dual: bad argument");
    PackParams p1 = pack2d(d_x, rows, cols, cols);
    p1.Rp = (int)rows; p1.Kp = (int)cols_padded; p1.C = 1; p1.scales = d_scale; p1.qm1 = (float)(qmax - 1);
    PackParams p2 = p1;
    p1.dst = d_q1; p2.dst = d_q2;
    if (sos) {
        p1.mode = PACK_SOS_HI; p2.mode = PACK_SOS_LO;
    } else {
        p1.lo = 0; p1.hi = hi; p2.lo = lo; p2.hi = 0; p2.scales = nullptr; p2.neg_scale = const_scale;
    }
    if (!dual_pack_ok(p1, p2)) return fail(P4V_ERR_INVALID, "p4v_debug_pack_dual: not a dual pair");
    Ctx c{(hipStream_t)stream, Arena(nullptr, 0), false};
    const long total = rows * (cols_padded / 16);
    if (total >= (1L << 31)) return fail(P4V_ERR_UNSUPPORTED, "p4v_debug_pack_dual: plane too large");
    return enqueue(c, KERN(PackDualParams, k_pack_dual), dim3((unsigned)std::min<long>(cdiv(total, 256), 256L * 64)), dim3(256), 0,
                   PackDualParams{p1, p2});
}

int p4v_debug_pack_cands(const float* d_x, long rows, long cols, long rows_padded, long cols_padded, int layout, int lo, int hi,
                         const float* d_scales, int n_cands, const int* d_crange, const unsigned char* d_done, int live_max,
                         int general, int8_t* d_q, void* stream) {
    if (!d_x || !d_scales || !d_q || rows <= 0 || cols <= 0 || rows_padded < rows || cols_padded % 64 || cols_padded < cols ||
        layout < 0 || layout > 3 || (layout == 3 && rows_padded % 64) || lo > hi || lo < -128 || hi > 127 || n_cands <= 0 ||
        (d_done && !d_crange) || (live_max >= 0 && !d_crange))
        return fail(P4V_ERR_INVALID, "p4v_debug_pack_cands: bad argument");
    Ctx c{(hipStream_t)stream, Arena(nullptr, 0), false};
    cvt_bias(c);
    PackParams p = pack2d(d_x, rows, cols, cols);
    p.Rp = (int)rows_padded; p.Kp = (int)cols_padded; p.dst = d_q; p.C = n_cands; p.c_inner = layout;
    p.scales = d_scales; p.sc_cs = 1; p.lo = lo; p.hi = hi;
    p.crange = d_crange; p.c_base = 0; p.done = d_done;
    g_pack_general.store(general ? 1 : 0, std::memory_order_relaxed);
    const int r = launch_pack<int8_t>(c, p, live_max);
    g_pack_general.store(0, std::memory_order_relaxed);
    return r;
}

int p4v_debug_prep_epi6(const float* d_o, const float* d_wt, const float* d_bias, long o_ss, long o_ts, int sr, int tr,
                        int bias_on_t, int wt_mode, int transposed, float* d_e, void* stream) {
// ... 65 lines not shown
```

### ptq4vit_amd/csrc/p4v_kernels.h

```cpp
#pragma once
#include <hip/hip_runtime.h>
#include <stdint.h>
#include <type_traits>

namespace p4v {

typedef int v4i __attribute__((ext_vector_type(4)));
typedef int v16i __attribute__((ext_vector_type(16)));
typedef float v4f __attribute__((ext_vector_type(4)));
typedef float v16f __attribute__((ext_vector_type(16)));
typedef float v2f __attribute__((ext_vector_type(2)));

#ifndef P4V_GROUP_KERNARG
#define P4V_GROUP_KERNARG (4096 - 256)
#endif
template <typename P> struct GroupArgs {
    static constexpr int CAP_RAW = (P4V_GROUP_KERNARG - 16) / (int)(sizeof(P) + 16);
    static constexpr int CAP = CAP_RAW > 64 ? 64 : CAP_RAW;
    int n;
    unsigned off[CAP + 1];
    unsigned gx[CAP], gy[CAP], gz[CAP];
    P p[CAP];
};
#define P4V_BIDX uint3{blockIdx.x, blockIdx.y, blockIdx.z}
#define P4V_GDIM uint3{gridDim.x, gridDim.y, gridDim.z}
#define P4V_GROUP_ENTER(a)                                                                           \
    int m_ = 0;                                                                                      \
    while (m_ + 1 < a.n && blockIdx.x >= a.off[m_ + 1]) ++m_;                                        \
    m_ = __builtin_amdgcn_readfirstlane(m_);                                                         \
    const unsigned b_ = blockIdx.x - a.off[m_];                                                      \
    const uint3 vg_{a.gx[m_], a.gy[m_], a.gz[m_]};                                                   \
    if (b_ >= vg_.x * vg_.y * vg_.z) return;                                                         \
    const uint3 vb_{b_ % vg_.x, (b_ / vg_.x) % vg_.y, b_ / (vg_.x * vg_.y)}

__device__ __forceinline__ unsigned enc_ordered(float f) {
    unsigned b = __float_as_uint(f);
    return (b & 0x80000000u) ? ~b : (b | 0x80000000u);
}
__device__ __forceinline__ float dec_ordered(unsigned e) {
    unsigned b = (e & 0x80000000u) ? (e & 0x7fffffffu) : ~e;
    return __uint_as_float(b);
}

struct AbsMaxParams {
    const float* src;
    long s0, s1, s2, s3;
    int D0, D1, R, C;
    int nV, nH, crb_r, crb_c;
    int row_tile;
    int signed_max;
    unsigned* out;
};

__device__ __forceinline__ void k_absmax_body(const AbsMaxParams& p, const uint3 blockIdx, const uint3 gridDim) {
    int bx = blockIdx.x;
    const int h = bx % p.nH; bx /= p.nH;
    const int v = bx % p.nV; bx /= p.nV;
    const int rt = bx;
    const int r0 = v * p.crb_r + rt * p.row_tile;
    const int r1 = min(min(r0 + p.row_tile, (v + 1) * p.crb_r), p.R);
    const int c0 = h * p.crb_c;
    const int c1 = min(c0 + p.crb_c, p.C);
    const int w = c1 - c0;
    const float* base = p.src + (long)blockIdx.z * p.s0 + (long)blockIdx.y * p.s1;
    float m = -INFINITY;
    if (w > 0 && r1 > r0 && p.s3 == 1 && (w & 3) == 0 && (p.s2 & 3) == 0 && (c0 & 3) == 0 && ((((unsigned long long)base) & 15) == 0)) {
        const int w4 = w >> 2;
        const int tpr = w4 >= 256 ? 256 : w4 >= 128 ? 128 : w4 >= 64 ? 64 : w4 >= 32 ? 32 : 16;
        const int tx = threadIdx.x & (tpr - 1), ty = threadIdx.x / tpr, rpar = 256 / tpr;
        for (int r = r0 + ty; r < r1; r += rpar) {
            const v4f* row = reinterpret_cast<const v4f*>(base + (long)r * p.s2 + c0);
            for (int c = tx; c < w4; c += tpr) {
                const v4f x = row[c];
                if (p.signed_max) m = fmaxf(fmaxf(m, fmaxf(x[0], x[1])), fmaxf(x[2], x[3]));
                else m = fmaxf(fmaxf(m, fmaxf(fabsf(x[0]), fabsf(x[1]))), fmaxf(fabsf(x[2]), fabsf(x[3])));
            }
        }
    } else if (w > 0 && r1 > r0) {
        const int n = (r1 - r0) * w;
        for (int i = threadIdx.x; i < n; i += 256) {
            const int r = r0 + i / w, c = c0 + i % w;
            float x = base[(long)r * p.s2 + (long)c * p.s3];
            m = fmaxf(m, p.signed_max ? x : fabsf(x));
        }
    }
    for (int o = 32; o > 0; o >>= 1) m = fmaxf(m, __shfl_xor(m, o));
    __shared__ float red[4];
    if ((threadIdx.x & 63) == 0) red[threadIdx.x >> 6] = m;
    __syncthreads();
    if (threadIdx.x == 0) {
        m = fmaxf(fmaxf(red[0], red[1]), fmaxf(red[2], red[3]));
        if (m > -INFINITY) atomicMax(p.out + ((long)blockIdx.y * p.nV + v) * p.nH + h, enc_ordered(m));
    }
}
// ... 440 lines not shown
        const int kc = (int)(i - row * kchunks);
        const int z = (int)(row / (unsigned)p.Rp);
        const int r = (int)(row - (unsigned)z * p.Rp);
        const float* zbase = p.zdiv > 0 ? p.src + (long)(z / p.zdiv) * p.s_z2 + (long)(z % p.zdiv) * p.s_z
                                        : p.src + (long)z * p.s_z;
        float x[16];
        pack_load16(p, zbase, r, kc, x);
        const bool live = r < p.R;
        int w1[4], w2[4];
#pragma unroll
        for (int q = 0; q < 4; ++q) {
            int a1 = 0, a2 = 0;
#pragma unroll
            for (int e = 0; e < 4; ++e) {
                const bool in = live && kc * 16 + q * 4 + e < p.K;
                const float v1 = in ? pack_value(p, x[q * 4 + e], s1) : 0.0f;
                const float v2 = in ? pack_value(p2, x[q * 4 + e], s2) : 0.0f;
                a1 |= ((int)v1 & 0xff) << (8 * e);
                a2 |= ((int)v2 & 0xff) << (8 * e);
            }
            w1[q] = a1; w2[q] = a2;
        }
        const long o = ((long)z * p.Rp + r) * p.Kp + (long)kc * 16;
        __builtin_nontemporal_store(v4i{w1[0], w1[1], w1[2], w1[3]}, reinterpret_cast<v4i*>(reinterpret_cast<int8_t*>(p.dst) + o));
        __builtin_nontemporal_store(v4i{w2[0], w2[1], w2[2], w2[3]}, reinterpret_cast<v4i*>(reinterpret_cast<int8_t*>(p2.dst) + o));
    }
}
__global__ __launch_bounds__(256) void k_pack_dual(PackDualParams p) { k_pack_dual_body(p, P4V_BIDX, P4V_GDIM); }
__global__ __launch_bounds__(256) void k_pack_dual_g(GroupArgs<PackDualParams> a) { P4V_GROUP_ENTER(a); k_pack_dual_body(a.p[m_], vb_, vg_); }

__global__ void k_fake_quant_rows(const float* x, long rows, long cols, const float* scales, long rows_per_scale,
                                  float lo, float hi, float* y) {
    const long n = rows * cols;
    for (long i = (long)blockIdx.x * blockDim.x + threadIdx.x; i < n; i += (long)gridDim.x * blockDim.x) {
        const float s = scales[(i / cols) / rows_per_scale];
        y[i] = fminf(fmaxf(rintf(x[i] / s), lo), hi) * s;
    }
}

__global__ __launch_bounds__(256) void k_multi_copy(const long* table, long index) {
    const long* e = table + 3 * (long)blockIdx.y;
    const char* src = reinterpret_cast<const char*>(e[0]);
    const long bytes = e[2];
    char* dst = reinterpret_cast<char*>(e[1]) + index * bytes;
    if (((e[0] | (long)(size_t)dst | bytes) & 15) == 0) {
        const long n = bytes >> 4;
        for (long i = (long)blockIdx.x * 256 + threadIdx.x; i < n; i += (long)gridDim.x * 256)
            reinterpret_cast<v4i*>(dst)[i] = reinterpret_cast<const v4i*>(src)[i];
    } else {
        const long n = bytes >> 2;
        for (long i = (long)blockIdx.x * 256 + threadIdx.x; i < n; i += (long)gridDim.x * 256)
            reinterpret_cast<int*>(dst)[i] = reinterpret_cast<const int*>(src)[i];
    }
}

enum ExportMode {
    EXP_SYM_I8 = 0,
    EXP_SYM_F32 = 1,
    EXP_GELU_U8 = 2,
    EXP_SOS_U8 = 3
};

struct ExportParams {
    const float* src; long ss[4]; int d[4];
    const float* s1; long s1s[4]; int s1d[4];
    const float* s2; long s2s[4]; int s2d[4]; float s2_const;
    int mode, lo1, hi1, lo2, hi2; float qm1;
    void* dst;
};

__global__ __launch_bounds__(256) void k_export(ExportParams p) {
    const long n3 = p.d[3], n23 = (long)p.d[2] * n3, n123 = (long)p.d[1] * n23, total = (long)p.d[0] * n123;
    for (long i = (long)blockIdx.x * 256 + threadIdx.x; i < total; i += (long)gridDim.x * 256) {
        const int i0 = (int)(i / n123), i1 = (int)((i % n123) / n23), i2 = (int)((i % n23) / n3), i3 = (int)(i % n3);
        const float x = p.src[i0 * p.ss[0] + i1 * p.ss[1] + i2 * p.ss[2] + i3 * p.ss[3]];
        const float s1 = p.s1[(i0 / p.s1d[0]) * p.s1s[0] + (i1 / p.s1d[1]) * p.s1s[1] + (i2 / p.s1d[2]) * p.s1s[2] + (i3 / p.s1d[3]) * p.s1s[3]];
        const float s2 = p.s2 ? p.s2[(i0 / p.s2d[0]) * p.s2s[0] + (i1 / p.s2d[1]) * p.s2s[1] + (i2 / p.s2d[2]) * p.s2s[2] + (i3 / p.s2d[3]) * p.s2s[3]]
                              : p.s2_const;
        if (p.mode == EXP_SYM_I8 || p.mode == EXP_SYM_F32) {
            const float q = fminf(fmaxf(rintf(x / s1), (float)p.lo1), (float)p.hi1);
            if (p.mode == EXP_SYM_I8) reinterpret_cast<int8_t*>(p.dst)[i] = (int8_t)(int)q;
            else reinterpret_cast<float*>(p.dst)[i] = q;
        } else if (p.mode == EXP_GELU_U8) {
            const float pos = fminf(fmaxf(rintf(x / s1), 0.0f), (float)p.hi1);
            const float neg = fabsf(fminf(fmaxf(rintf(x / s2), (float)p.lo2), 0.0f));
            reinterpret_cast<uint8_t*>(p.dst)[i] = (uint8_t)(((int)pos + 128 + (int)neg) & 0xff);
        } else {
            const float hi = fminf(fmaxf(rintf(fminf(fmaxf(x, s1), 1.0f) * p.qm1), 0.0f), p.qm1);
            const float lo = fminf(fmaxf(rintf(fminf(fmaxf(x, 0.0f), s1) / s2), 0.0f), p.qm1);
            reinterpret_cast<uint8_t*>(p.dst)[i] = (uint8_t)(((int)hi + 128 + (int)lo) & 0xff);
        }
    }
}

enum EpiMode {
    EPI_SQ_W = 0,
    EPI_SQ = 1,
    EPI_ABS = 2,
    EPI_W_SQ = 3,
    EPI_COS = 4,
    EPI_STORE = 5
    ,EPI_FWD = 6
    ,EPI_COS_T = 7
};

__device__ __forceinline__ void clip_crange(const int* crange, int& lo, int& hi, bool even = false) {
// ... 2879 lines not shown
    double norm;
    float* scores;
};
__device__ __forceinline__ float cos_item(const FinishCosParams& p, int c, int zb, int zv0, int zv1, int smp) {
    float dot = 0.f, nn = 0.f, oo = 0.f;
    for (int zv = zv0; zv < zv1; ++zv)
        for (int f = 0; f < p.FS; ++f) {
            const float* q = p.part + (long)c * p.p_cs + (long)(zb * p.ZV + zv) * p.p_zs + ((long)f * p.Sp + smp) * 3;
            dot += q[0]; nn += q[1]; oo += q[2];
        }
    const float na = fmaxf(sqrtf(oo), 1e-8f), nb = fmaxf(sqrtf(nn), 1e-8f);
    return dot / (na * nb);
}
__device__ __forceinline__ void k_finish_cos_body(const FinishCosParams& p, const uint3 blockIdx, const uint3 gridDim) {
    const int c = blockIdx.x, j = blockIdx.y, nt = blockDim.x;
    double acc = 0.0;
    if (p.j_mode == 3) {
        const int smp = j * nt + threadIdx.x;
        if (smp < p.S) {
            for (int zb = 0; zb < p.ZB; ++zb) acc += (double)cos_item(p, c, zb, 0, p.ZV, smp);
            p.scores[(long)c * p.nj + smp] = (float)(p.norm * acc);
        }
        return;
    }
    int zv0 = 0, zv1 = p.ZV, zlo = 0, zstep = 1;
    if (p.j_mode == 1) { zv0 = j; zv1 = j + 1; }
    if (p.j_mode == 2) { zlo = j; zstep = p.j_div; }
    const int nz = (p.ZB - zlo + zstep - 1) / zstep;
    const long total = (long)nz * p.S;
    for (long i = threadIdx.x; i < total; i += nt) {
        const int smp = (int)(i % p.S);
        const int zb = zlo + (int)(i / p.S) * zstep;
        acc += (double)cos_item(p, c, zb, zv0, zv1, smp);
    }
    __shared__ double red[1024];
    red[threadIdx.x] = acc;
    __syncthreads();
    for (int o = nt >> 1; o > 0; o >>= 1) {
        if (threadIdx.x < o) red[threadIdx.x] += red[threadIdx.x + o];
        __syncthreads();
    }
    if (threadIdx.x == 0) p.scores[(long)c * p.nj + j] = (float)(p.norm * red[0]);
}
__global__ __launch_bounds__(1024) void k_finish_cos(FinishCosParams p) { k_finish_cos_body(p, P4V_BIDX, P4V_GDIM); }
__global__ __launch_bounds__(1024) void k_finish_cos_g(GroupArgs<FinishCosParams> a) { P4V_GROUP_ENTER(a); k_finish_cos_body(a.p[m_], vb_, vg_); }

struct RowMassParams { const float* W; const float* O; long rows; long cols; int wt_mode; float* mass; };
__device__ __forceinline__ void k_row_mass_body(const RowMassParams& a_, const uint3 blockIdx, const uint3 gridDim) {
    const auto& [W, O, rows, cols, wt_mode, mass] = a_;
    const long r = (long)blockIdx.x * 4 + (threadIdx.x >> 6);
    if (r >= rows) return;
    const int lane = threadIdx.x & 63;
    const float* src = (wt_mode == 1 ? W : O) + r * cols;
    float s = 0.0f;
    if (wt_mode == 0) s = lane == 0 ? 1.0f : 0.0f;
    else
        for (long i = lane; i < cols; i += 64) {
            const float v = src[i];
            s += wt_mode == 2 ? fabsf(v) : v * v;
        }
    for (int o = 32; o > 0; o >>= 1) s += __shfl_xor(s, o);
    if (lane == 0) mass[r] = s;
}
__global__ __launch_bounds__(256) void k_row_mass(RowMassParams p) { k_row_mass_body(p, P4V_BIDX, P4V_GDIM); }
__global__ __launch_bounds__(256) void k_row_mass_g(GroupArgs<RowMassParams> a) { P4V_GROUP_ENTER(a); k_row_mass_body(a.p[m_], vb_, vg_); }
__global__ void k_group_mass(const float* mass, int n_groups, int group, float* out) {
    const int g = blockIdx.x * blockDim.x + threadIdx.x;
    if (g >= n_groups) return;
    float s = 0.0f;
    for (int i = 0; i < group; ++i) s += mass[(long)g * group + i];
    out[g] = s;
}
struct TopkParams { const float* mass_all; int n; int k; int* idx_all; };
__device__ __forceinline__ void k_topk_rows_body(const TopkParams& a_, const uint3 blockIdx, const uint3 gridDim) {
    const auto& [mass_all, n, k, idx_all] = a_;
    const float* mass = mass_all + (long)blockIdx.x * n;
    int* idx = idx_all + (long)blockIdx.x * k;
    __shared__ int hist[256];
    __shared__ int wtot[4];
    __shared__ int wg[2][16], we[2][16];
    __shared__ unsigned prefix_s;
    __shared__ int krem_s;
    const int t = threadIdx.x, lane = t & 63, wv = t >> 6;
    auto key = [&](int i) -> unsigned { const unsigned b = __float_as_uint(mass[i]); return (b & 0x80000000u) ? 0u : b; };
    if (t == 0) { prefix_s = 0; krem_s = k; }
    for (int shift = 24; shift >= 0; shift -= 8) {
        if (t < 256) hist[t] = 0;
        __syncthreads();
        const unsigned hi_mask = shift == 24 ? 0u : (0xFFFFFFFFu << (shift + 8));
        const unsigned pre = prefix_s;
        const int kr = krem_s;
        for (int i0 = 0; i0 < n; i0 += 1024) {
            const int i = i0 + t;
            const unsigned kv = i < n ? key(i) : 0u;
            const bool in = i < n && (kv & hi_mask) == pre;
            const int d = (int)((kv >> shift) & 255u);
            const unsigned long long m = __ballot(in);
            if (m) {
                const int d0 = __shfl(d, __ffsll((long long)m) - 1);
                if (__ballot(in && d != d0) == 0ull) { if (lane == __ffsll((long long)m) - 1) atomicAdd(&hist[d0], __popcll(m)); }
                else if (in) atomicAdd(&hist[d], 1);
            }
        }
        __syncthreads();
        const int h = t < 256 ? hist[t] : 0;
        int sfx = h;
        for (int o = 1; o < 64; o <<= 1) { const int v = __shfl_down(sfx, o); if (lane + o < 64) sfx += v; }
        if (t < 256 && lane == 0) wtot[wv] = sfx;
        __syncthreads();
        if (t < 256) {
            int above = 0;
            for (int q = wv + 1; q < 4; ++q) above += wtot[q];
            const int incl = sfx + above, excl = incl - h;
            if (excl < kr && kr <= incl) { prefix_s = pre | ((unsigned)t << shift); krem_s = kr - excl; }
// ... 136 lines not shown
```

### ptq4vit_amd/engine.py

```python
import ctypes as C

import torch

from . import _lib

_workspace = {}
_mult_cache = {}


def _require_cuda(t, what):
    if not t.is_cuda:
        raise RuntimeError(f"ptq4vit_amd: {what} must live on the GPU (got {t.device}); the calibration path has no CPU fallback")


def device_of(*tensors):
    for t in tensors:
        if t is not None and t.is_cuda:
            return t.device
    if not torch.cuda.is_available():
        raise RuntimeError("ptq4vit_amd: no GPU visible -- the HIP calibration engine needs an MI355X (no CPU fallback)")
    return torch.device("cuda", torch.cuda.current_device())


def to_dev(t, dev):
# ... 12 lines not shown
        ws = torch.empty(int(nbytes) + pad, dtype=torch.uint8, device=dev)
        _workspace[key] = ws
    return ws


def release_workspace():
    _workspace.clear()


def workspace_bytes(dev=None):
    return sum(ws.numel() for (d, _s, _slot), ws in _workspace.items() if dev is None or d == dev)


def workspace_held(dev, slot=0):
    ws = _workspace.get((dev, torch.cuda.current_stream(dev).cuda_stream, slot))
    return 0 if ws is None else ws.numel()


_side_streams = {}


def side_streams(dev, n):
    lst = _side_streams.setdefault(dev, [])
    while len(lst) < n:
        lst.append(torch.cuda.Stream(device=dev))
    return lst[:n]


def candidate_multipliers(eq_alpha, eq_beta, eq_n, dev):
    key = (float(eq_alpha), float(eq_beta), int(eq_n), str(dev))
    t = _mult_cache.get(key)
    if t is None:
        t = torch.tensor([eq_alpha + i * (eq_beta - eq_alpha) / eq_n for i in range(eq_n + 1)],
                         dtype=torch.float32).to(dev)
        _mult_cache[key] = t
    return t


def ptr(t):
    return C.c_void_p(t.data_ptr()) if t is not None else C.c_void_p(0)


def stream_ptr(dev):
    return C.c_void_p(torch.cuda.current_stream(dev).cuda_stream)


def metric_id(name):
    if name not in _lib.METRICS:
        raise NotImplementedError(f"metric {name} not implemented!")
    return _lib.METRICS[name]


class Job:
    __slots__ = ("kind", "name", "desc", "inputs", "mult", "outputs", "need", "dev", "scores", "best")

    def __init__(self, kind, name, desc, inputs, mult, outputs, need, dev, scores=None, best=None):
        self.kind, self.name, self.desc, self.inputs, self.mult = kind, name, desc, inputs, mult
        self.outputs, self.need, self.dev, self.scores, self.best = outputs, need, dev, scores, best


def _need(fn, desc, what):
    need = fn(C.byref(desc))
    if need == 0:
        _lib.check(-1 if not _lib.load().p4v_last_error() else -2, what)
    return need


def run_job(job):
    lib = _lib.load()
    ws = workspace(job.dev, job.need)
    with torch.cuda.device(job.dev):
        rc = getattr(lib, job.name)(C.byref(job.desc), *[ptr(t) for t in job.inputs], ptr(job.mult), *[ptr(t) for t in job.outputs],
                                    ptr(job.scores), ptr(job.best), ptr(ws), ws.numel(), stream_ptr(job.dev))
    _lib.check(rc, job.name)
    return job


def calibrate_group(jobs, inputs_ready=None):
    jobs = list(jobs)
    if not jobs:
        return jobs
    lib = _lib.load()
    dev = jobs[0].dev
    arr = (_lib.GroupJob * len(jobs))()
    offs, total = [], 0
    for job in jobs:
        offs.append(total)
        total += (int(job.need) + 4095) & ~4095
    arena = workspace(dev, total, slot="arena")
    base = arena.data_ptr()
    keep = [arena]
    for i, job in enumerate(jobs):
        if job.dev != dev:
            raise ValueError("calibrate_group: every member must live on the same device")
        if job.scores is not None:
            raise ValueError("calibrate_group: score tables are only returned by the single-module calls")
        g = arr[i]
        g.kind, g.status, g.desc = job.kind, 0, C.cast(C.pointer(job.desc), C.c_void_p)
        ins = list(job.inputs) + [None] * (5 - len(job.inputs))
        for k in range(5):
            g.inp[k] = ins[k].data_ptr() if ins[k] is not None else None
        g.mult = job.mult.data_ptr()
        outs = list(job.outputs) + [None] * (3 - len(job.outputs))
        for k in range(3):
            g.out[k] = outs[k].data_ptr() if outs[k] is not None else None
        g.workspace, g.workspace_bytes = base + offs[i], int(job.need)
    with torch.cuda.device(dev):
        ev = C.c_void_p(inputs_ready.cuda_event) if inputs_ready is not None else C.c_void_p(0)
        rc = lib.p4v_calibrate_group(arr, len(jobs), stream_ptr(dev), ev)
    _lib.check(rc, "p4v_calibrate_group")
    del keep
    return jobs


def launch_counters(reset=False):
    out = (C.c_int64 * 4)()
    _lib.check(_lib.load().p4v_launch_counters(out, int(bool(reset))), "p4v_launch_counters")
    return dict(zip(("asked", "issued", "rounds", "groups"), (int(v) for v in out)))


def linear_job(*, weight, bias, x, out, grad, w_bit, a_bit, metric, eq_alpha, eq_beta, eq_n, search_round,
               n_V, n_H, n_a, init_layerwise=False, postgelu=False, want_scores=False, force_f32=False, memoize=True,
               prune=True):
    lib = _lib.load()
    dev = device_of(x, weight)
    weight, bias, x, out, grad = (to_dev(t, dev) for t in (weight, bias, x, out, grad))
    x = x.contiguous(); out = out.contiguous(); weight = weight.contiguous()
    grad = grad.contiguous() if grad is not None else None
    batch = x.shape[0]
    K = x.shape[-1]
    tokens = x.numel() // (batch * K)
    N = weight.shape[0]
    d = _lib.LinearDesc(batch, tokens, K, N, n_V, n_H, n_a, w_bit, a_bit, metric_id(metric), eq_n, search_round,
                        int(postgelu), int(init_layerwise), int(bias is not None),
                        int(force_f32) | (0 if memoize else 2) | (0 if prune else 8))
    need = _need(lib.p4v_linear_workspace_bytes, d, "p4v_linear_workspace_bytes")
    mult = candidate_multipliers(eq_alpha, eq_beta, eq_n, dev)
    w_iv = torch.empty(n_V * n_H, dtype=torch.float32, device=dev)
    a_iv = torch.empty(n_a, dtype=torch.float32, device=dev)
    scores = torch.zeros(search_round, 2, eq_n, n_V, dtype=torch.float32, device=dev) if want_scores else None
    best = torch.zeros(search_round, 2, n_V, dtype=torch.int32, device=dev) if want_scores else None
    return Job(_lib.JOB_LINEAR, "p4v_linear_calibrate", d, (weight, bias, x, out, grad), mult, (w_iv, a_iv), need, dev, scores, best)


def linear_calibrate(**kw):
    job = run_job(linear_job(**kw))
    return job.outputs[0], job.outputs[1], job.scores, job.best


def linear_quant_forward(*, weight, bias, x, w_interval, a_interval, w_bit, a_bit, n_V, n_H, n_a, postgelu=False):
    lib = _lib.load()
    dev = device_of(x, weight)
    weight, bias, x = (to_dev(t, dev) for t in (weight, bias, x))
    x = x.contiguous(); weight = weight.contiguous()
    batch, K = x.shape[0], x.shape[-1]
    tokens = x.numel() // (batch * K)
    N = weight.shape[0]
    d = _lib.LinearDesc(batch, tokens, K, N, n_V, n_H, n_a, w_bit, a_bit, metric_id("L2_norm"), 1, 1,
                        int(postgelu), 0, int(bias is not None), 4)
    need = lib.p4v_linear_workspace_bytes(C.byref(d))
    if need == 0:
        _lib.check(-2, "p4v_linear_workspace_bytes")
# ... 299 lines not shown
    x2d = x2d.contiguous().float()
    rows, cols = x2d.shape
    y = torch.empty_like(x2d)
    scales = scales.to(x2d.device, torch.float32).reshape(-1).contiguous()
    with torch.cuda.device(x2d.device):
        rc = lib.p4v_fake_quant(ptr(x2d), rows, cols, ptr(scales), int(rows_per_scale), int(lo), int(hi), ptr(y),
                                stream_ptr(x2d.device))
    _lib.check(rc, "p4v_fake_quant")
    return y


def _pad4(seq, fill):
    seq = list(seq)
    return [fill] * (4 - len(seq)) + seq


def export_quantize(src, *, mode, scale1, scale1_stride, scale1_div, lo1=0, hi1=0, scale2=None, scale2_stride=(0, 0, 0, 0),
                    scale2_div=(1, 1, 1, 1), scale2_const=0.0, lo2=0, hi2=0, qmax=128, dims=None, src_stride=None):
    lib = _lib.load()
    _require_cuda(src, "export source")
    dev = src.device
    src = src.detach()
    if src.dtype != torch.float32:
        if src_stride is not None and not src.is_contiguous():
            raise TypeError("export_quantize: explicit src_stride needs a float32 source (convert before deriving the strides)")
        src = src.float()
    if dims is None:
        dims, src_stride = _pad4(src.shape, 1), _pad4(src.stride(), 0)
    code = {"sym_i8": _lib.EXPORT_SYM_I8, "sym_f32": _lib.EXPORT_SYM_F32, "gelu_u8": _lib.EXPORT_GELU_U8,
            "sos_u8": _lib.EXPORT_SOS_U8}[mode]
    out = torch.empty(tuple(dims), dtype={"sym_i8": torch.int8, "sym_f32": torch.float32}.get(mode, torch.uint8), device=dev)
    d = _lib.ExportDesc()
    for i in range(4):
        d.dims[i], d.src_stride[i] = int(dims[i]), int(src_stride[i])
        d.scale1_stride[i], d.scale1_div[i] = int(scale1_stride[i]), int(scale1_div[i])
        d.scale2_stride[i], d.scale2_div[i] = int(scale2_stride[i]), int(scale2_div[i])
    d.scale2_const = float(scale2_const)
    d.mode, d.lo1, d.hi1, d.lo2, d.hi2, d.qmax, d.reserved = code, int(lo1), int(hi1), int(lo2), int(hi2), int(qmax), 0
    s1 = to_dev(torch.as_tensor(scale1), dev).reshape(-1).contiguous()
    s2 = to_dev(torch.as_tensor(scale2), dev).reshape(-1).contiguous() if scale2 is not None else None
    with torch.cuda.device(dev):
        rc = lib.p4v_export_quantize(C.byref(d), ptr(src), ptr(s1), ptr(s2), ptr(out), stream_ptr(dev))
    _lib.check(rc, "p4v_export_quantize")
    return out


def multi_copy(table, n, index, max_bytes, dev):
    lib = _lib.load()
    with torch.cuda.device(dev):
        rc = lib.p4v_multi_copy(ptr(table), int(n), int(index), int(max_bytes), stream_ptr(dev))
    _lib.check(rc, "p4v_multi_copy")


def stats_enable(flag):
    _lib.load().p4v_stats_enable(int(bool(flag)))


def debug_variant(variant=0, force_generic=False):
    _lib.check(_lib.load().p4v_debug_set_variant(int(variant), int(bool(force_generic))), "p4v_debug_set_variant")


def debug_tuning(key, value):
    _lib.check(_lib.load().p4v_debug_set_tuning(int(key), int(value)), "p4v_debug_set_tuning")


def debug_topk_rows(mass, k):
    assert mass.is_cuda and mass.dtype == torch.float32 and mass.dim() == 2 and mass.is_contiguous()
    segs, n = mass.shape
    out = torch.empty(segs, int(k), dtype=torch.int32, device=mass.device)
    with torch.cuda.device(mass.device):
        rc = _lib.load().p4v_debug_topk_rows(ptr(mass), segs, n, int(k), ptr(out), stream_ptr(mass.device))
    _lib.check(rc, "p4v_debug_topk_rows")
    return out


def debug_pack_dual(x2d, *, sos, scale, lo, hi, qmax, const_scale=0.0):
    x2d = x2d.contiguous().float()
    rows, cols = x2d.shape
    colsp = (cols + 63) // 64 * 64
    q1 = torch.empty(rows, colsp, dtype=torch.int8, device=x2d.device)
    q2 = torch.empty_like(q1)
    sc = torch.tensor([float(scale)], dtype=torch.float32, device=x2d.device)
    with torch.cuda.device(x2d.device):
        rc = _lib.load().p4v_debug_pack_dual(ptr(x2d), rows, cols, colsp, int(bool(sos)), int(lo), int(hi), int(qmax), ptr(sc),
                                             float(const_scale), ptr(q1), ptr(q2), stream_ptr(x2d.device))
    _lib.check(rc, "p4v_debug_pack_dual")
    return q1[:, :cols], q2[:, :cols], q1, q2


def debug_pack_cands(x2d, scales, *, layout, lo, hi, rows_padded=None, crange=None, done=None, live_max=-1, general=False,
                     out=None):
    x2d = x2d.contiguous().float()
    scales = scales.contiguous().float()
    rows, cols = x2d.shape
    n = scales.numel()
    colsp = (cols + 63) // 64 * 64
    rowsp = rows if rows_padded is None else int(rows_padded)
    size = rowsp * colsp * (1 if layout == 3 else (n + 1) // 2 * 2 if layout == 2 else n)
    if out is None:
        out = torch.zeros(size, dtype=torch.int8, device=x2d.device)
    assert out.dtype == torch.int8 and out.is_contiguous() and out.numel() >= size
    with torch.cuda.device(x2d.device):
        rc = _lib.load().p4v_debug_pack_cands(ptr(x2d), rows, cols, rowsp, colsp, int(layout), int(lo), int(hi), ptr(scales), n,
                                              ptr(crange) if crange is not None else None,
                                              ptr(done) if done is not None else None, int(live_max), int(bool(general)),
                                              ptr(out), stream_ptr(x2d.device))
# ... 40 lines not shown
```

### ptq4vit_amd/utils/quant_calib.py

```python
import os
import sys

import torch
import torch.nn.functional as F

from ..quant_layers.conv import MinMaxQuantConv2d
from ..quant_layers.linear import MinMaxQuantLinear
from ..quant_layers.matmul import MinMaxQuantMatMul
from . import shard

try:
    from tqdm import tqdm
except Exception:
    def tqdm(x, **k):
        return x


_HWQ_WARNED = False


def _warn_hw_queues(n_streams):
    global _HWQ_WARNED
    if _HWQ_WARNED or n_streams <= 1 or os.environ.get("GPU_MAX_HW_QUEUES"):
        return
# ... 43 lines not shown
    module.raw_input[0].append(input[0].detach())
    module.raw_input[1].append(input[1].detach())
    module.raw_out.append(output.detach())


def _register(module, with_grad):
    hooks = []
    wrap = _with_output_grad if with_grad else (lambda h: h)
    if isinstance(module, MinMaxQuantLinear):
        hooks.append(module.register_forward_hook(wrap(linear_forward_hook)))
    if isinstance(module, MinMaxQuantConv2d):
        hooks.append(module.register_forward_hook(wrap(conv2d_forward_hook)))
    if isinstance(module, MinMaxQuantMatMul):
        hooks.append(module.register_forward_hook(wrap(matmul_forward_hook)))
    return hooks


def _concat(module, with_grad):
    cat = lambda t: t[0] if len(t) == 1 else torch.cat(t, dim=0)
    if isinstance(module, MinMaxQuantMatMul):
        module.raw_input = [cat(t) for t in module.raw_input]
    else:
        module.raw_input = cat(module.raw_input)
    module.raw_out = cat(module.raw_out)
    if with_grad:
        module.raw_grad = cat(module.raw_grad)


def _cache_like(t, n_sub):
    shape = (n_sub * t.shape[0],) + tuple(t.shape[1:])
    if t.is_contiguous() or t.dim() < 2:
        return torch.empty(shape, dtype=t.dtype, device=t.device)
    order = sorted(range(t.dim()), key=lambda k: (-t.stride(k), k))
    dense, expect = order[0] == 0, 1
    for k in reversed(order):
        dense &= t.stride(k) == expect
        expect *= t.shape[k]
    if not dense:
        return torch.empty(shape, dtype=t.dtype, device=t.device)
    strides, acc = [0] * t.dim(), 1
    for k in reversed(order):
        strides[k] = acc
        acc *= shape[k]
    return torch.empty_strided(shape, strides, dtype=t.dtype, device=t.device)


def _same_dense_block(cache, t):
    if t.element_size() != 4 or cache.dtype != t.dtype:
        return False
    if tuple(cache.stride()[1:]) != tuple(t.stride()[1:]) or cache.stride(0) != t.stride(0):
        return False
    span = 1 + sum((t.shape[k] - 1) * t.stride(k) for k in range(t.dim()))
    return span == t.numel() and t.stride(0) == max(t.stride())


def _groupable(m):
    if "calibration_step2" in m.__dict__ or not hasattr(m, "calibration_job"):
        return False
    return getattr(getattr(type(m), "calibration_step2", None), "_p4v_grouped", False)


class QuantCalibrator:

    def __init__(self, net, wrapped_modules, calib_loader, sequential=True):
        self.net = net
        self.wrapped_modules = wrapped_modules
        self.calib_loader = calib_loader
        self.sequential = sequential
        self.calibrated = False

    def _run_loader(self):
        dev = _dev_of(self.net)
        with torch.no_grad():
            for inp, _ in self.calib_loader:
                self.net(inp.to(dev))

    def sequential_quant_calib(self):
        for step in range(2):
            print(f"Start calibration step={step + 1}")
            for module in self.wrapped_modules.values():
                if hasattr(module, "calibrated"):
                    if step == 1:
                        module.mode = "raw"
                else:
                    module.mode = f"calibration_step{step + 1}"
            self._run_loader()
        for module in self.wrapped_modules.values():
            module.mode = "quant_forward"
        print("sequential calibration finished")

    def parallel_quant_calib(self):
        print("Start calibration step=1")
        for module in self.wrapped_modules.values():
            module.mode = "raw" if hasattr(module, "calibrated") else "calibration_step1"
        self._run_loader()
        dev = _dev_of(self.net)
        for name, module in tqdm(self.wrapped_modules.items(), desc="Calibration"):
            if hasattr(module, "calibrated"):
                continue
            module.mode = "calibration_step2"
            with torch.no_grad():
                if isinstance(module, MinMaxQuantMatMul):
                    module.forward(module.raw_input[0].to(dev), module.raw_input[1].to(dev))
                else:
                    module.forward(module.raw_input.to(dev))
        for module in self.wrapped_modules.values():
# ... 232 lines not shown
        import time
        trace = os.environ.get("P4V_CAPTURE_TRACE") == "1"

        def tick(label, t_prev):
            if not trace:
                return t_prev
            torch.cuda.synchronize(dev)
            now = time.time()
            print(f"[capture] {label}: {now - t_prev:.3f} s", file=sys.stderr, flush=True)
            return now
        t_ = time.time()
        cache = self.net.__dict__.setdefault("_p4v_capture_graphs", {})
        key = self._graph_key(dev, bs, inp)
        lanes = cache.get(key)
        shadow = self.net.__dict__.get("_p4v_capture_shadow") if lanes is not None else None
        if shadow is not None and lanes is shadow.get("lanes"):
            self._sync_shadow(shadow)
        else:
            shadow = None
        if lanes is None:
            seen_before = self.net.__dict__.get("_p4v_calibrations", 0) > 0
            shadow = self._arch_shadow(dev, bs, inp, build=bool(use_graph or n_sub >= 24 or seen_before))
            if shadow is not None:
                lanes = shadow["lanes"]
                if not lanes:
                    entry = self._build_graph(dev, bs, inp, raw_pred_softmax, shadow)
                    if entry is None:
                        shadow["net"] = None
                        lanes = shadow = None
                    else:
                        lanes.append(entry)
            if shadow is not None:
                cache.clear()
                cache[key] = lanes
                self.net.__dict__["_p4v_capture_shadow"] = shadow
        if lanes is None:
            seen_before = self.net.__dict__.get("_p4v_calibrations", 0) > 0
            if not (use_graph or n_sub >= 24 or seen_before):
                return False
            entry = self._build_graph(dev, bs, inp, raw_pred_softmax)
            if entry is None:
                return False
            cache.clear()
            lanes = cache[key] = [entry]
        want = int(getattr(self, "capture_lanes", None) or os.environ.get("P4V_CAPTURE_LANES", "3"))
        while len(lanes) < max(1, min(want, n_sub)):
            entry = self._build_graph(dev, bs, inp, raw_pred_softmax, shadow)
            if entry is None:
                break
            lanes.append(entry)
        n_lanes = max(1, min(want, n_sub, len(lanes)))
        t_ = tick(f"graphs ready ({len(lanes)} instance(s))", t_)
        from .. import engine
        flat_dsts, plans = [], []
        key_names = tuple(names)
        recipe0 = lanes[0].setdefault("recipes", {}).get(key_names)
        if recipe0 is None:
            statics0 = lanes[0]["statics"]
            layout, is_block = [], []
            for n in names:
                for t in statics0[n][0]:
                    c = _cache_like(t, n_sub)
                    layout.append((tuple(c.shape), tuple(c.stride()), t.dtype))
                    is_block.append(_same_dense_block(c, t))
                    del c
            recipe0 = lanes[0]["recipes"][key_names] = {"n_sub": n_sub, "layout": layout, "is_block": is_block}
        if recipe0["n_sub"] != n_sub:
            lanes[0]["recipes"].pop(key_names)
            return self._capture_passes_graph(names, dev, bs, raw_pred_softmax)
        k_ = 0
        for n in names:
            m = self.wrapped_modules[n]
            stat, with_g = lanes[0]["statics"][n]
            full = []
            for _t in stat:
                shp, strd, dt = recipe0["layout"][k_]
                full.append(torch.empty_strided(shp, strd, dtype=dt, device=dev))
                k_ += 1
            d_ = m.__dict__
            if isinstance(m, MinMaxQuantMatMul):
                d_["raw_input"], d_["raw_out"] = [full[0], full[1]], full[2]
            else:
                d_["raw_input"], d_["raw_out"] = full[0], full[1]
            if hasattr(m, "metric"):
                d_["raw_grad"] = full[-1] if with_g else None
            flat_dsts += full
        for li in range(n_lanes):
            statics = lanes[li]["statics"]
            srcs = []
            for n in names:
                srcs += statics[n][0]
            lane_blocks = lanes[li].setdefault("is_block", {}).get(key_names)
            if lane_blocks is None:
                lane_blocks = [bool(b) and _same_dense_block(d, t) for d, t, b in zip(flat_dsts, srcs, recipe0["is_block"])]
                lanes[li]["is_block"][key_names] = lane_blocks
            block = [(d, t) for d, t, b in zip(flat_dsts, srcs, lane_blocks) if b]
            other = [(d, t) for d, t, b in zip(flat_dsts, srcs, lane_blocks) if not b]
            table, max_bytes = None, 0
            if block:
                rows = [[t.data_ptr(), d.data_ptr(), t.numel() * 4] for d, t in block]
                table = torch.tensor(rows, dtype=torch.int64).to(dev, non_blocking=True)
                max_bytes = max(r[2] for r in rows)
            plans.append((lanes[li], table, len(block), max_bytes, other))
        t_ = tick(f"caches allocated ({sum(d.numel() * 4 for d in flat_dsts) / 2**30:.1f} GiB)", t_)
        main = torch.cuda.current_stream(dev)
        streams = [main] if n_lanes == 1 else engine.side_streams(dev, n_lanes)
        for s_ in streams:
            if s_ is not main:
                s_.wait_stream(main)
        for i, st in enumerate(range(0, total, bs)):
            entry, table, n_block, max_bytes, other = plans[i % n_lanes]
            with torch.cuda.stream(streams[i % n_lanes]):
                with torch.no_grad():
                    entry["in"].copy_(inp[st:st + bs])
                entry["tgt"].copy_(raw_pred_softmax[st:st + bs])
                entry["graph"].replay()
                if table is not None:
                    engine.multi_copy(table, n_block, i, max_bytes, dev)
                    if i < n_lanes:
                        table.record_stream(streams[i % n_lanes])
                for d, t in other:
                    d[i * t.shape[0]:(i + 1) * t.shape[0]].copy_(t)
        for s_ in streams:
            if s_ is not main:
                main.wait_stream(s_)
        tick(f"{n_sub} replays + appends on {n_lanes} stream(s)", t_)
        return True

    def _capture_passes(self, dev, bs, raw_pred_softmax, with_grad, stride=None):
        i = -1
        for inp, _ in self.calib_loader:
            total = inp.shape[0]
            for st in range(0, total, bs):
                i += 1
                if stride is not None and i % stride[1] != stride[0]:
                    continue
                inp_ = inp[st:st + bs].to(dev)
                if with_grad:
                    inp_ = inp_.detach().requires_grad_(True)
                    inv_n = self._inv_rows(total, st, inp_.shape[0], self._ref_bs(), dev)
                    self._kl_loss(self.net(inp_), raw_pred_softmax[st:st + bs], inv_n).backward()
                else:
                    with torch.no_grad():
                        self.net(inp_)

    def _search_concurrent(self, names, n_streams):
        import threading
        import time
        dev = _dev_of(self.net)
        main = torch.cuda.current_stream(dev)
        from .. import engine
        _warn_hw_queues(n_streams)
        streams = engine.side_streams(dev, n_streams)
        if not hasattr(self, "_module_ms"):
            self._module_ms = {}
        for s in streams:
            s.wait_stream(main)
        keep = [(m.raw_input, m.raw_out, getattr(m, "raw_grad", None)) for m in (self.wrapped_modules[n] for n in names)]
        todo = list(names)
        measured = (self.net.__dict__.get("_p4v_module_ms") or {}).get("ms", {})
        if os.environ.get("P4V_SEARCH_ORDER", "lpt") == "lpt" and all(n in measured for n in names):
            todo.sort(key=lambda n: measured[n], reverse=True)
        elif os.environ.get("P4V_SEARCH_ORDER", "lpt") == "lpt":
            def work(n):
                m = self.wrapped_modules[n]
                ri = m.raw_input
                if isinstance(ri, (list, tuple)):
                    a, b = ri
                    return float(a.numel()) * b.shape[-1] * (0.2 if a.shape[-1] <= 64 else 1.0)
                w = getattr(m, "weight", None)
                return float(ri.numel()) / max(1, ri.shape[-1] if ri.dim() != 4 else 1) * (w.numel() if w is not None else 1) / (1 if ri.dim() != 4 else ri.shape[1])
# ... 57 lines not shown
        if not early:
            inputs_ready = None
            for s in streams:
                s.wait_stream(main)
        keep = [(m.raw_input, m.raw_out, getattr(m, "raw_grad", None)) for m in (self.wrapped_modules[n] for n in names)]
        def kind(n):
            m = self.wrapped_modules[n]
            ri = m.raw_input
            shp = tuple(tuple(t.shape) for t in ri) if isinstance(ri, (list, tuple)) else tuple(ri.shape)
            return (type(m).__name__, shp, tuple(m.raw_out.shape))
        order = sorted(names, key=lambda n: (str(kind(n)), names.index(n)))
        parts = [order[i::n_calls] for i in range(n_calls)]
        budget_all = int(float(os.environ.get("P4V_GROUP_GIB", "150")) * (1 << 30))
        if dev.type == "cuda":
            free, _tot = torch.cuda.mem_get_info(dev)
            pooled = torch.cuda.memory_reserved(dev) - torch.cuda.memory_allocated(dev)
            avail = int(free + pooled) + engine.workspace_bytes(dev) - (6 << 30)
            if avail < budget_all:
                engine.release_workspace()
                budget_all = max(4 << 30, avail)
        budget = budget_all // n_calls
        errors = []

        def cost(n, sizes):
            return shard.module_cost_ms(self.wrapped_modules[n], sizes[n])

        def worker(s, part):
            try:
                torch.cuda.set_device(dev)
                with torch.cuda.stream(s), torch.no_grad():
                    todo = list(part)
                    while todo and not errors:
                        t_grp = time.perf_counter()
                        batch, jobs, sizes, acc = [], [], {}, 0
                        while todo:
                            n = todo[0]
                            m = self.wrapped_modules[n]
                            if not _groupable(m):
                                if batch:
                                    break
                                todo.pop(0)
                                m.calibration_step2()
                                m.mode = "raw"
                                self._module_ms[n] = (time.perf_counter() - t_grp) * 1e3
                                t_grp = time.perf_counter()
                                continue
                            ri = m.raw_input
                            sizes[n] = 4 * (sum(t.numel() for t in ri) if isinstance(ri, (list, tuple)) else ri.numel()) + 8 * m.raw_out.numel()
                            job = m.calibration_job()
                            held = (int(job.need) + 4095) & ~4095
                            if batch and acc + held > budget:
                                break
                            todo.pop(0)
                            batch.append(n); jobs.append(job); acc += held
                        if not batch:
                            continue
                        engine.calibrate_group(jobs, inputs_ready=inputs_ready)
                        for n, j in zip(batch, jobs):
                            m = self.wrapped_modules[n]
                            m.calibration_install(j)
                            m.mode = "raw"
                        ms = (time.perf_counter() - t_grp) * 1e3
                        w = {n: cost(n, sizes) for n in batch}
                        tot = sum(w.values()) or 1.0
                        for n in batch:
                            self._module_ms[n] = ms * w[n] / tot
            except BaseException as e:
                errors.append(e)

        if n_calls == 1:
            worker(streams[0], parts[0])
        else:
            threads = [threading.Thread(target=worker, args=(s, p)) for s, p in zip(streams, parts)]
            for t in threads:
                t.start()
            for t in threads:
                t.join()
        for s in streams:
            main.wait_stream(s)
        torch.cuda.synchronize(dev)
        del keep
        if errors:
            raise errors[0]

    def _estimate_cache_bytes(self, names):
        dev = _dev_of(self.net)
        geom = None
        for inp, _ in self.calib_loader:
            geom = (tuple(inp.shape[1:]), int(inp.shape[0]), tuple(self.wrapped_modules))
            break
        memo = self.net.__dict__.setdefault("_p4v_cache_sizes", {})
        if geom in memo and all(n in memo[geom] for n in names):
            return {n: memo[geom][n] for n in names}
        arch = (type(self.net).__name__, str(dev), geom,
                tuple((n, tuple(p_.shape)) for n, p_ in self.net.named_parameters()),
                tuple((n, type(m).__name__) for n, m in self.wrapped_modules.items()))
        known = HessianQuantCalibrator._ARCH_SIZES.get(arch)
        if known is not None and all(n in known[0] for n in names):
            for n, mn in known[1].items():
                if n in self.wrapped_modules:
                    self.wrapped_modules[n]._p4v_out_mn = mn
            memo.setdefault(geom, {}).update(known[0])
            return {n: known[0][n] for n in names}
        sizes = {}
        hooks = []

# ... 69 lines not shown
        replay_is_cheap = (with_grad and dev_.type == "cuda" and not self.sequential and getattr(self, "use_graph", None) is not False
                           and len(list(self.calib_loader)) == 1
                           and (getattr(self, "use_graph", None) is True or n_sub >= 24 or self.net.__dict__.get("_p4v_calibrations", 0) > 0
                                or bool(self.net.__dict__.get("_p4v_capture_graphs"))))
        budget = self._resolve_budget(replay_is_cheap)

        def plan(todo, budget_):
            if self.sequential:
                return [[n] for n in todo]
            if shard_cap:
                return [todo]
            sizes = all_sizes if all_sizes is not None else self._estimate_cache_bytes(todo)
            out, cur, acc = [], [], 0
            for n in todo:
                if cur and acc + sizes.get(n, 0) > budget_:
                    out.append(cur)
                    cur, acc = [], 0
                cur.append(n)
                acc += sizes.get(n, 0)
            if cur:
                out.append(cur)
            return out

        def run_group(grp):
            t1 = time.time()
            n_streams = getattr(self, "search_streams", None) or int(os.environ.get("P4V_SEARCH_STREAMS", "4"))
            grouped = getattr(self, "search_grouped", None)
            if grouped is None:
                grouped = os.environ.get("P4V_GROUPED", "1") != "0"
            concurrent = batching and not self.sequential and (n_streams > 1 or grouped) and _dev_of(self.net).type == "cuda" and len(grp) > 1
            cap_done = None
            if shard_cap:
                self._capture(names, raw_pred_softmax, with_grad, stride=(rank, world))
                grad_names = {n for n in names if with_grad and hasattr(self.wrapped_modules[n], "metric")}
                shard.exchange_captures(self.wrapped_modules, owner, n_sub, grad_names)
            else:
                self._capture(grp, raw_pred_softmax, with_grad)
            if concurrent and not shard_cap and os.environ.get("P4V_CAPTURE_SYNC", "0") != "1":
                dev_g = _dev_of(self.net)
                cap_done = torch.cuda.Event(enable_timing=True)
                cap_done.record(torch.cuda.current_stream(dev_g))
            elif torch.cuda.is_available():
                torch.cuda.synchronize()
            t2 = time.time()
            if concurrent:
                if grouped:
                    calls = 1 if n_streams == 1 else (getattr(self, "group_calls", None) or int(os.environ.get("P4V_GROUP_CALLS", "0")))
                    if calls <= 0:
                        small = sum(self._estimate_cache_bytes(grp).values()) < (512 << 20)
                        calls = 1 if small else 3
                    self._search_grouped(grp, calls, inputs_ready=cap_done)
                else:
                    self._search_concurrent(grp, n_streams)
                if cap_done is not None:
                    ref = torch.cuda.Event(enable_timing=True)
                    ref.record(torch.cuda.current_stream(_dev_of(self.net)))
                    ref.synchronize()
                    t_end = time.time()
                    t2 = max(t2, t_end - cap_done.elapsed_time(ref) * 1e-3)
            else:
                for n in tqdm(grp, desc="Hessian"):
                    module = self.wrapped_modules[n]
                    with torch.no_grad():
                        if batching:
                            module.calibration_step2()
                        elif isinstance(module, MinMaxQuantMatMul):
                            module.calibration_step2(module.raw_input[0], module.raw_input[1])
                        else:
                            module.calibration_step2(module.raw_input)
                    module.mode = "quant_forward" if self.sequential else "raw"
            if torch.cuda.is_available():
                torch.cuda.synchronize()
            return t2 - t1, time.time() - t2

        if world > 1 and not self.sequential and want_shard:
            per_rank = [sum(all_sizes.get(n, 0) for n in names if owner[n] == r) for r in range(world)]
            during = sum(all_sizes.values()) / world
            shard_budget = self.cache_budget_bytes if self.cache_budget_bytes is not None else (200 << 30)
            shard_cap = (n_sub >= world and 2 * max(per_rank) + 2 * during <= shard_budget
                         and all(inp.shape[0] % bs_ == 0 for inp, _ in self.calib_loader))
            self.capture_mode = "sharded" if shard_cap else "replicated"
        groups = plan(mine, budget)
        t_cap = t_cal = 0.0
        done = set()
        while groups:
            grp = groups.pop(0)
            try:
                dc, ds = run_group(grp)
            except torch.cuda.OutOfMemoryError as oom:
                if os.environ.get("P4V_CAPTURE_TRACE", "0") == "1":
                    import traceback
                    tb = traceback.extract_tb(oom.__traceback__)
                    print("[ptq4vit_amd] OOM at " + " <- ".join(f"{os.path.basename(f.filename)}:{f.lineno}({f.name})" for f in tb[-4:]) + ": " + str(oom).split("\n")[0][:200], flush=True)
                if shard_cap or len(grp) <= 1:
                    raise
                from .. import engine
                for n in grp:
                    m = self.wrapped_modules[n]
                    if n not in done and not (hasattr(m, "calibrated") and not hasattr(m, "raw_out")):
                        m.raw_input = m.raw_out = None
                        if hasattr(m, "metric"):
                            m.raw_grad = None
                engine.release_workspace()
                torch.cuda.empty_cache()
                budget //= 2
                print(f"[ptq4vit_amd] out of memory with {len(grp)} modules resident: retrying with a cache budget of {budget >> 30} GiB")
# ... 26 lines not shown
```

Before: 664.7.

## Fuse absmax and gradient row-mass stats into capture copy and reuse in calibration

Capture-time copies now go through a new append kernel that, while copying activations and gradients into the calibration cache, also accumulates per-tensor absolute/signed max and per-row gradient mass into a small stats arena. The grouped calibration entry point takes these precomputed stats and skips the separate absmax and row-mass kernels when pointers and shapes match. This avoids re-reading large cached tensors, at the cost of atomics in the copy kernel, more plan and bookkeeping code, and pointer-matching checks that fall back to the old path on any mismatch.

```diff
diff --git a/include/ptq4vit_hip.h b/include/ptq4vit_hip.h
--- a/include/ptq4vit_hip.h
+++ b/include/ptq4vit_hip.h
@@ -8,7 +8,7 @@
 extern "C" {
 #endif
 
-#define P4V_VERSION 140
+#define P4V_VERSION 141
 
 enum p4v_metric {
     P4V_METRIC_L1_NORM = 0,
@@ -108,6 +108,15 @@
 } p4v_group_job;
 int p4v_calibrate_group(p4v_group_job* jobs, int32_t n_jobs, void* stream, void* inputs_ready_event);
 
+typedef struct p4v_group_stats {
+    const uint32_t* max_a;
+    const uint32_t* max_b;
+    const float* row_mass;
+    int64_t mass_rows, mass_cols;
+} p4v_group_stats;
+int p4v_calibrate_group_stats(p4v_group_job* jobs, const p4v_group_stats* stats, int32_t n_jobs, void* stream,
+                              void* inputs_ready_event);
+
 int p4v_launch_counters(int64_t* out4, int reset);
 
 
@@ -200,6 +209,9 @@
                              size_t workspace_bytes, void* stream);
 
 int p4v_multi_copy(const int64_t* d_table, int32_t n, int64_t index, int64_t max_bytes, void* stream);
+
+enum p4v_append_kind { P4V_APPEND_NONE = 0, P4V_APPEND_ABSMAX = 1, P4V_APPEND_MAX = 2, P4V_APPEND_ROW_MASS = 3 };
+int p4v_capture_append(const int64_t* d_table, int32_t n, int64_t index, int64_t max_bytes, void* stream);
 
 typedef struct p4v_kernel_stats {
     double sweep_i8_ms;
diff --git a/include/ptq4vit_hip_debug.h b/include/ptq4vit_hip_debug.h
--- a/include/ptq4vit_hip_debug.h
+++ b/include/ptq4vit_hip_debug.h
@@ -10,6 +10,8 @@
 int p4v_debug_set_variant(int variant, int force_generic);
 int p4v_debug_set_tuning(int key, int value);
 int p4v_debug_topk_rows(const float* d_mass, int segs, int n, int k, int32_t* d_idx, void* stream);
+int p4v_debug_row_mass(const float* d_grad, int64_t rows, int64_t cols, float* d_mass, void* stream);
+int p4v_debug_stats_skipped(int64_t* out2, int reset);
 int p4v_debug_pack_dual(const float* d_x, long rows, long cols, long cols_padded, int sos, int lo, int hi, int qmax,
                         const float* d_scale, float const_scale, int8_t* d_q1, int8_t* d_q2, void* stream);
 int p4v_debug_pack_cands(const float* d_x, long rows, long cols, long rows_padded, long cols_padded, int layout, int lo, int hi,
diff --git a/ptq4vit_amd/_lib.py b/ptq4vit_amd/_lib.py
--- a/ptq4vit_amd/_lib.py
+++ b/ptq4vit_amd/_lib.py
@@ -74,7 +74,13 @@
                 ("out", C.c_void_p * 3), ("workspace", C.c_void_p), ("workspace_bytes", C.c_size_t)]
 
 
+class GroupStats(C.Structure):
+    _fields_ = [("max_a", C.c_void_p), ("max_b", C.c_void_p), ("row_mass", C.c_void_p), ("mass_rows", C.c_int64), ("mass_cols", C.c_int64)]
+
+
 JOB_LINEAR, JOB_MATMUL, JOB_CONV = 0, 1, 2
+APPEND_NONE, APPEND_ABSMAX, APPEND_MAX, APPEND_ROW_MASS = 0, 1, 2, 3
+APPEND_MAX_UNITS = 256
 PLANE_SYM, PLANE_SOS_HI, PLANE_SOS_LO, PLANE_TWIN = 1, 2, 3, 4
 EXPORT_SYM_I8, EXPORT_SYM_F32, EXPORT_GELU_U8, EXPORT_SOS_U8 = 0, 1, 2, 3
 
@@ -84,16 +90,16 @@
     "p4v_linear_workspace_bytes", "p4v_linear_calibrate",
     "p4v_matmul_workspace_bytes", "p4v_matmul_calibrate",
     "p4v_conv_workspace_bytes", "p4v_conv_calibrate",
-    "p4v_calibrate_group", "p4v_launch_counters",
+    "p4v_calibrate_group", "p4v_calibrate_group_stats", "p4v_launch_counters",
     "p4v_linear_quant_forward", "p4v_matmul_quant_forward",
     "p4v_amax_init_linear", "p4v_linear_search_w", "p4v_linear_search_a",
     "p4v_amax_init_matmul", "p4v_matmul_search_A", "p4v_sos_search_split", "p4v_matmul_search_B",
     "p4v_amax_init_conv", "p4v_conv_search_w_channelwise", "p4v_conv_search_w_layerwise", "p4v_conv_search_a",
     "p4v_score_argmax_gather",
-    "p4v_quantize_i8", "p4v_pack_plane_i8", "p4v_fake_quant", "p4v_export_quantize", "p4v_multi_copy",
+    "p4v_quantize_i8", "p4v_pack_plane_i8", "p4v_fake_quant", "p4v_export_quantize", "p4v_multi_copy", "p4v_capture_append",
     "p4v_stats_enable", "p4v_stats_reset", "p4v_stats_get", "p4v_stats_launches", "p4v_prune_counters",
     "p4v_debug_set_variant", "p4v_debug_set_tuning", "p4v_debug_topk_rows", "p4v_debug_pack_dual", "p4v_debug_prep_epi6",
-    "p4v_debug_pack_cands",
+    "p4v_debug_pack_cands", "p4v_debug_row_mass", "p4v_debug_stats_skipped",
 ]
 
 _lib = None
@@ -158,6 +164,12 @@
     lib.p4v_export_quantize.argtypes = [C.POINTER(ExportDesc), fp, fp, fp, vp, vp]
     lib.p4v_multi_copy.restype = C.c_int
     lib.p4v_multi_copy.argtypes = [vp, C.c_int32, C.c_int64, C.c_int64, vp]
+    lib.p4v_capture_append.restype = C.c_int
+    lib.p4v_capture_append.argtypes = [vp, C.c_int32, C.c_int64, C.c_int64, vp]
+    lib.p4v_debug_row_mass.restype = C.c_int
+    lib.p4v_debug_row_mass.argtypes = [fp, C.c_int64, C.c_int64, fp, vp]
+    lib.p4v_debug_stats_skipped.restype = C.c_int
+    lib.p4v_debug_stats_skipped.argtypes = [C.POINTER(C.c_int64), C.c_int]
     lib.p4v_debug_topk_rows.restype = C.c_int
     lib.p4v_debug_topk_rows.argtypes = [vp, C.c_int, C.c_int, C.c_int, vp, vp]
     lib.p4v_debug_pack_dual.restype = C.c_int
@@ -184,6 +196,8 @@
     lib.p4v_launch_counters.argtypes = [C.POINTER(C.c_int64), C.c_int]
     lib.p4v_calibrate_group.restype = C.c_int
     lib.p4v_calibrate_group.argtypes = [C.POINTER(GroupJob), C.c_int32, vp, vp]
+    lib.p4v_calibrate_group_stats.restype = C.c_int
+    lib.p4v_calibrate_group_stats.argtypes = [C.POINTER(GroupJob), C.POINTER(GroupStats), C.c_int32, vp, vp]
     _lib = lib
     return lib
 
diff --git a/ptq4vit_amd/csrc/p4v_api.hip b/ptq4vit_amd/csrc/p4v_api.hip
--- a/ptq4vit_amd/csrc/p4v_api.hip
+++ b/ptq4vit_amd/csrc/p4v_api.hip
@@ -100,7 +100,14 @@
     Group* grp = nullptr;
     int slot = 0;
     int par = 1;
+    const p4v_group_stats* pre = nullptr;
+    const float* pre_grad = nullptr;
 };
+std::atomic<long long> g_pre_cnt[2];
+inline const unsigned* pre_max(const Ctx& c, int which) {
+    if (!c.pre) return nullptr;
+    return reinterpret_cast<const unsigned*>(which == 0 ? c.pre->max_a : c.pre->max_b);
+}
 
 struct StatInfo { int kind; double macs, alg; int stage, gx, gz; double bytes; };
 struct QOp;
@@ -1266,15 +1273,20 @@
     const void* wsrc = g.G ? (const void*)g.G : (const void*)g.O;
     const bool new_idx = sc->idx_src != wsrc || sc->idx_wt != g.wt_mode || (g.wt_mode != 1 && sc->o_src != g.O);
     if (new_idx) {
-        CHK(enqueue(c, KERN(RowMassParams, k_row_mass), dim3((unsigned)cdiv(zrows, 4)), dim3(256), 0, RowMassParams{g.G ? g.G : g.O, g.O, zrows, (long)g.Ncols, g.wt_mode, sc->mass}));
-        CHK(enqueue(c, KERN(TopkParams, k_topk_rows), dim3(g.segs), dim3(1024), 0, TopkParams{sc->mass, g.seg_rows, g.k, sc->idx}));
+        const float* mass = sc->mass;
+        if (c.pre && c.pre->row_mass && g.wt_mode == 1 && g.G && g.G == c.pre_grad && zrows == c.pre->mass_rows && (long)g.Ncols == c.pre->mass_cols) {
+            mass = c.pre->row_mass;
+            g_pre_cnt[1].fetch_add(1, std::memory_order_relaxed);
+        } else
+            CHK(enqueue(c, KERN(RowMassParams, k_row_mass), dim3((unsigned)cdiv(zrows, 4)), dim3(256), 0, RowMassParams{g.G ? g.G : g.O, g.O, zrows, (long)g.Ncols, g.wt_mode, sc->mass}));
+        CHK(enqueue(c, KERN(TopkParams, k_topk_rows), dim3(g.segs), dim3(1024), 0, TopkParams{mass, g.seg_rows, g.k, sc->idx}));
         sc->idx_src = wsrc; sc->idx_wt = g.wt_mode;
         sc->o_src = sc->g_src = sc->r_src = nullptr;
         if (sc->frac && host_sync_ok && !(g_variant & 8388608)) {
             float f = 1.0f;
             int* hm = host_mirror(c);
             CHK(enqueue(c, KERN(MassFracParams, k_mass_fraction), dim3(1), dim3(1024), 0,
-                        MassFracParams{sc->mass, zrows, sc->idx, g.segs, g.seg_rows, g.k, sc->frac, hm ? reinterpret_cast<float*>(hm + 4) : nullptr}));
+                        MassFracParams{mass, zrows, sc->idx, g.segs, g.seg_rows, g.k, sc->frac, hm ? reinterpret_cast<float*>(hm + 4) : nullptr}));
             if (!hm) CHK(q_d2h(c, &f, sc->frac, sizeof f));
             CHK(q_sync(c));
             if (hm) f = *reinterpret_cast<volatile float*>(hm + 4);
@@ -1858,8 +1870,10 @@
     auto init_activation_side = [&]() -> int {
         if (!fwd_out && (sg.mask & ST_INIT)) {
             const long stw[4] = {0, 0, K, 1};
-            CHK(launch_absmax(c, X, stw, 1, 1, M, K, 1, nA, M, crb_acts, d->twin_postgelu ? 1 : 0, enc_a));
-            CHK(launch_interval(c, enc_a, nA, (float)(aq - 0.5), d->init_layerwise, a_iv));
+            const unsigned* pm = nA == 1 ? pre_max(c, 0) : nullptr;
+            if (pm) { if (!c.dry) g_pre_cnt[0].fetch_add(1, std::memory_order_relaxed); }
+            else CHK(launch_absmax(c, X, stw, 1, 1, M, K, 1, nA, M, crb_acts, d->twin_postgelu ? 1 : 0, enc_a));
+            CHK(launch_interval(c, pm ? pm : enc_a, nA, (float)(aq - 0.5), d->init_layerwise, a_iv));
             if (sg.searches()) CHK(launch_cands(c, mult, a_iv, ncand, nA, a_cands_ws));
         }
         return 0;
@@ -2120,10 +2134,14 @@
         const long sa[4] = {d->a_stride[0], d->a_stride[1], d->a_stride[2], d->a_stride[3]};
         const long sb[4] = {d->b_stride[0], d->b_stride[1], d->b_stride[2], d->b_stride[3]};
         float* a_dst = d->sos ? A_headwise : A_iv;
-        CHK(launch_absmax(c, A, sa, d->batch, H, M, K, 1, 1, M, K, 0, enc_A));
-        CHK(launch_interval(c, enc_A, H, (float)(Aq - 0.5), d->init_layerwise, a_dst));
-        CHK(launch_absmax(c, B, sb, d->batch, H, K, N, 1, 1, K, N, 0, enc_B));
-        CHK(launch_interval(c, enc_B, H, (float)(Bq - 0.5), d->init_layerwise, B_iv));
+        const unsigned* pmA = pre_max(c, 0);
+        const unsigned* pmB = pre_max(c, 1);
+        if (pmA) { if (!c.dry) g_pre_cnt[0].fetch_add(1, std::memory_order_relaxed); }
+        else CHK(launch_absmax(c, A, sa, d->batch, H, M, K, 1, 1, M, K, 0, enc_A));
+        CHK(launch_interval(c, pmA ? pmA : enc_A, H, (float)(Aq - 0.5), d->init_layerwise, a_dst));
+        if (pmB) { if (!c.dry) g_pre_cnt[0].fetch_add(1, std::memory_order_relaxed); }
+        else CHK(launch_absmax(c, B, sb, d->batch, H, K, N, 1, 1, K, N, 0, enc_B));
+        CHK(launch_interval(c, pmB ? pmB : enc_B, H, (float)(Bq - 0.5), d->init_layerwise, B_iv));
         if (sg.searches()) {
             if (!d->sos) CHK(launch_cands(c, mult, A_iv, ncand, H, A_cands_ws));
             CHK(launch_cands(c, mult, B_iv, ncand, H, B_cands_ws));
@@ -2334,8 +2352,10 @@
         CHK(launch_absmax(c, W, stw, 1, 1, oc, K, nw, 1, d->channelwise ? 1 : oc, K, 0, enc_w));
         CHK(launch_interval(c, enc_w, nw, (float)(wq - 0.5), d->init_layerwise, w_iv));
         const long stx[4] = {0, 0, (long)ic * H * Wd, 1};
-        CHK(launch_absmax(c, X, stx, 1, 1, b, ic * H * Wd, 1, 1, b, ic * H * Wd, 0, enc_a));
-        CHK(launch_interval(c, enc_a, 1, aquant ? (float)(aq - 0.5) : (float)(std::ldexp(1.0, d->a_bit - 1) - 0.5), 0, a_iv));
+        const unsigned* pm = pre_max(c, 0);
+        if (pm) { if (!c.dry) g_pre_cnt[0].fetch_add(1, std::memory_order_relaxed); }
+        else CHK(launch_absmax(c, X, stx, 1, 1, b, ic * H * Wd, 1, 1, b, ic * H * Wd, 0, enc_a));
+        CHK(launch_interval(c, pm ? pm : enc_a, 1, aquant ? (float)(aq - 0.5) : (float)(std::ldexp(1.0, d->a_bit - 1) - 0.5), 0, a_iv));
         if (sg.searches()) {
             CHK(launch_cands(c, mult, w_iv, ncand, nw, w_cands_ws));
             CHK(launch_cands(c, mult, a_iv, ncand, 1, a_cands_ws));
@@ -2599,6 +2619,10 @@
 
 
 int p4v_calibrate_group(p4v_group_job* jobs, int32_t n_jobs, void* stream, void* inputs_ready_event) {
+    return p4v_calibrate_group_stats(jobs, nullptr, n_jobs, stream, inputs_ready_event);
+}
+
+int p4v_calibrate_group_stats(p4v_group_job* jobs, const p4v_group_stats* stats, int32_t n_jobs, void* stream, void* inputs_ready_event) {
     if (n_jobs < 0 || (n_jobs > 0 && !jobs)) return fail(P4V_ERR_INVALID, "p4v_calibrate_group: bad job list");
     if (n_jobs == 0) return 0;
     for (int i = 0; i < n_jobs; ++i) {
@@ -2629,6 +2653,7 @@
             (void)hipSetDevice(dev);
             g_stat_on = g.stat_on; g_stage = 0; g_exec_frac = 1.0; g_memo_hits = 0; g_memo_misses = 0; g_err.clear();
             Ctx c{g.st, Arena(jobs[i].workspace, jobs[i].workspace_bytes), false, &g, i, par};
+            if (stats) { c.pre = &stats[i]; c.pre_grad = jobs[i].kind == P4V_JOB_MATMUL ? jobs[i].in[3] : jobs[i].in[4]; }
             const int r = run_group_member(jobs[i], c);
             jobs[i].status = r;
             if (r) errs[i] = g_err;
@@ -2811,6 +2836,15 @@
     const long n = rows * cols;
     hipLaunchKernelGGL(k_fake_quant_rows, dim3((unsigned)std::min<long>(cdiv(n, 256), 65536)), dim3(256), 0,
                        (hipStream_t)stream, d_x, (long)rows, (long)cols, d_scales, (long)rows_per_scale, (float)lo, (float)hi, d_y);
+    HIPCHK(hipGetLastError());
+    return 0;
+}
+
+int p4v_capture_append(const int64_t* d_table, int32_t n, int64_t index, int64_t max_bytes, void* stream) {
+    if (!d_table || n <= 0 || index < 0 || max_bytes <= 0) return fail(P4V_ERR_INVALID, "p4v_capture_append: bad argument");
+    static_assert(sizeof(long) == sizeof(int64_t), "table entries are 64-bit");
+    const unsigned gx = (unsigned)std::max<long>(1, std::min<long>(cdiv(max_bytes / 16, 256 * 8), 256));
+    hipLaunchKernelGGL(k_capture_append, dim3(gx, (unsigned)n), dim3(256), 0, (hipStream_t)stream, (const long*)d_table, (long)index);
     HIPCHK(hipGetLastError());
     return 0;
 }
@@ -2913,6 +2947,20 @@
     if (key < 0 || key >= 16) return fail(P4V_ERR_INVALID, "p4v_debug_set_tuning: unknown key %d", key);
     if (key == TUNE_B1_PATH && tune_b1_removed(value)) return fail(P4V_ERR_INVALID, "p4v_debug_set_tuning: 12 = %d selects a removed path", value);
     g_tune[key].store(value, std::memory_order_relaxed);
+    return 0;
+}
+
+int p4v_debug_row_mass(const float* d_grad, int64_t rows, int64_t cols, float* d_mass, void* stream) {
+    if (!d_grad || !d_mass || rows <= 0 || cols <= 0) return fail(P4V_ERR_INVALID, "p4v_debug_row_mass: bad argument");
+    hipLaunchKernelGGL(k_row_mass, dim3((unsigned)cdiv((long)rows, 4)), dim3(256), 0, (hipStream_t)stream,
+                       RowMassParams{d_grad, d_grad, (long)rows, (long)cols, 1, d_mass});
+    HIPCHK(hipGetLastError());
+    return 0;
+}
+
+int p4v_debug_stats_skipped(int64_t* out2, int reset) {
+    if (out2) for (int i = 0; i < 2; ++i) out2[i] = (int64_t)g_pre_cnt[i].load(std::memory_order_relaxed);
+    if (reset) for (int i = 0; i < 2; ++i) g_pre_cnt[i].store(0, std::memory_order_relaxed);
     return 0;
 }
 
diff --git a/ptq4vit_amd/csrc/p4v_kernels.h b/ptq4vit_amd/csrc/p4v_kernels.h
--- a/ptq4vit_amd/csrc/p4v_kernels.h
+++ b/ptq4vit_amd/csrc/p4v_kernels.h
@@ -40,6 +40,19 @@
 __device__ __forceinline__ float dec_ordered(unsigned e) {
     unsigned b = (e & 0x80000000u) ? (e & 0x7fffffffu) : ~e;
     return __uint_as_float(b);
+}
+
+__device__ __forceinline__ float row_mass_wave(const float* src, long cols, int wt_mode, int lane, float* copy) {
+#pragma clang fp contract(off)
+    float s = 0.0f;
+#pragma unroll 4
+    for (long i = lane; i < cols; i += 64) {
+        const float v = src[i];
+        if (copy) copy[i] = v;
+        s += wt_mode == 2 ? fabsf(v) : v * v;
+    }
+    for (int o = 32; o > 0; o >>= 1) s += __shfl_xor(s, o);
+    return s;
 }
 
 struct AbsMaxParams {
@@ -586,6 +599,104 @@
         for (long i = (long)blockIdx.x * 256 + threadIdx.x; i < n; i += (long)gridDim.x * 256)
             reinterpret_cast<int*>(dst)[i] = reinterpret_cast<const int*>(src)[i];
     }
+}
+
+enum { APPEND_NONE = 0, APPEND_ABSMAX = 1, APPEND_MAX = 2, APPEND_ROW_MASS = 3 };
+constexpr int APPEND_ROW = 8;
+constexpr int APPEND_MAX_UNITS = 256;
+
+template <int VW>
+__device__ __forceinline__ void append_copy_max(const char* src, char* dst, long n, bool signed_max, long chunk, int units, unsigned* smax) {
+    long w, stride, end;
+    unsigned r = 0, u = 0, sr = 0, su = 0;
+    const unsigned ch = (unsigned)chunk;
+    if (units > 1) {
+        const long per = (n + gridDim.x - 1) / gridDim.x;
+        w = (long)blockIdx.x * per;
+        end = w + per < n ? w + per : n;
+        w += threadIdx.x; stride = 256;
+        const long e0 = w * VW;
+        r = (unsigned)(e0 % chunk); u = (unsigned)((e0 / chunk) % units);
+        sr = (unsigned)((256L * VW) % chunk); su = (unsigned)(((256L * VW) / chunk) % units);
+    } else {
+        w = (long)blockIdx.x * 256 + threadIdx.x; stride = (long)gridDim.x * 256; end = n;
+    }
+    unsigned cur = 0;
+    float m = -INFINITY;
+    auto flush = [&] { if (m > -INFINITY) atomicMax(smax + cur, enc_ordered(m)); };
+    auto acc = [&](unsigned unit, float x) {
+        if (unit != cur) { flush(); cur = unit; m = -INFINITY; }
+        m = fmaxf(m, x);
+    };
+    for (; w < end; w += stride) {
+        if constexpr (VW == 4) {
+            const v4i x = reinterpret_cast<const v4i*>(src)[w];
+            reinterpret_cast<v4i*>(dst)[w] = x;
+            float f[4];
+#pragma unroll
+            for (int j = 0; j < 4; ++j) { f[j] = __int_as_float(x[j]); if (!signed_max) f[j] = fabsf(f[j]); }
+            if (units == 1 || r + 4 <= ch) acc(u, fmaxf(fmaxf(f[0], f[1]), fmaxf(f[2], f[3])));
+            else {
+                const unsigned un = u + 1 == (unsigned)units ? 0 : u + 1;
+#pragma unroll
+                for (int j = 0; j < 4; ++j) acc(r + j < ch ? u : un, f[j]);
+            }
+        } else {
+            const int x = reinterpret_cast<const int*>(src)[w];
+            reinterpret_cast<int*>(dst)[w] = x;
+            const float f = __int_as_float(x);
+            acc(u, signed_max ? f : fabsf(f));
+        }
+        if (units > 1) {
+            r += sr; u += su;
+            if (r >= ch) { r -= ch; ++u; }
+            if (u >= (unsigned)units) u -= (unsigned)units;
+        }
+    }
+    flush();
+}
+
+__global__ __launch_bounds__(256) void k_capture_append(const long* table, long index) {
+    const long* e = table + APPEND_ROW * (long)blockIdx.y;
+    const char* src = reinterpret_cast<const char*>(e[0]);
+    const long bytes = e[2];
+    char* dst = reinterpret_cast<char*>(e[1]) + index * bytes;
+    int kind = (int)e[3];
+    const long a = e[5], b = e[6];
+    __shared__ unsigned smax[APPEND_MAX_UNITS];
+    if (kind == APPEND_ROW_MASS && e[4] && a > 0 && b > 0 && a * b * 4 == bytes) {
+        float* mass = reinterpret_cast<float*>(e[4]) + index * b;
+        const int lane = threadIdx.x & 63;
+        for (long r = (long)blockIdx.x * 4 + (threadIdx.x >> 6); r < b; r += (long)gridDim.x * 4) {
+            const float s = row_mass_wave(reinterpret_cast<const float*>(src) + r * a, a, 1, lane, reinterpret_cast<float*>(dst) + r * a);
+            if (lane == 0) mass[r] = s;
+        }
+        return;
+    }
+    const bool with_max = (kind == APPEND_ABSMAX || kind == APPEND_MAX) && e[4] && b >= 1 && b <= APPEND_MAX_UNITS
+                          && (b == 1 || (a >= 4 && a < (1L << 31)));
+    const bool wide = ((e[0] | (long)(size_t)dst | bytes) & 15) == 0;
+    if (!with_max) {
+        if (wide) {
+            const long n = bytes >> 4;
+            for (long i = (long)blockIdx.x * 256 + threadIdx.x; i < n; i += (long)gridDim.x * 256)
+                reinterpret_cast<v4i*>(dst)[i] = reinterpret_cast<const v4i*>(src)[i];
+        } else {
+            const long n = bytes >> 2;
+            for (long i = (long)blockIdx.x * 256 + threadIdx.x; i < n; i += (long)gridDim.x * 256)
+                reinterpret_cast<int*>(dst)[i] = reinterpret_cast<const int*>(src)[i];
+        }
+        return;
+    }
+    const int units = (int)b;
+    for (int t = threadIdx.x; t < units; t += 256) smax[t] = 0;
+    __syncthreads();
+    if (wide) append_copy_max<4>(src, dst, bytes >> 4, kind == APPEND_MAX, a, units, smax);
+    else append_copy_max<1>(src, dst, bytes >> 2, kind == APPEND_MAX, a, units, smax);
+    __syncthreads();
+    unsigned* out = reinterpret_cast<unsigned*>(e[4]);
+    for (int t = threadIdx.x; t < units; t += 256)
+        if (smax[t]) atomicMax(out + t, smax[t]);
 }
 
 enum ExportMode {
@@ -3571,14 +3682,7 @@
     if (r >= rows) return;
     const int lane = threadIdx.x & 63;
     const float* src = (wt_mode == 1 ? W : O) + r * cols;
-    float s = 0.0f;
-    if (wt_mode == 0) s = lane == 0 ? 1.0f : 0.0f;
-    else
-        for (long i = lane; i < cols; i += 64) {
-            const float v = src[i];
-            s += wt_mode == 2 ? fabsf(v) : v * v;
-        }
-    for (int o = 32; o > 0; o >>= 1) s += __shfl_xor(s, o);
+    const float s = wt_mode == 0 ? 1.0f : row_mass_wave(src, cols, wt_mode, lane, nullptr);
     if (lane == 0) mass[r] = s;
 }
 __global__ __launch_bounds__(256) void k_row_mass(RowMassParams p) { k_row_mass_body(p, P4V_BIDX, P4V_GDIM); }
diff --git a/ptq4vit_amd/engine.py b/ptq4vit_amd/engine.py
--- a/ptq4vit_amd/engine.py
+++ b/ptq4vit_amd/engine.py
@@ -88,11 +88,12 @@
 
 
 class Job:
-    __slots__ = ("kind", "name", "desc", "inputs", "mult", "outputs", "need", "dev", "scores", "best")
+    __slots__ = ("kind", "name", "desc", "inputs", "mult", "outputs", "need", "dev", "scores", "best", "stats")
 
     def __init__(self, kind, name, desc, inputs, mult, outputs, need, dev, scores=None, best=None):
         self.kind, self.name, self.desc, self.inputs, self.mult = kind, name, desc, inputs, mult
         self.outputs, self.need, self.dev, self.scores, self.best = outputs, need, dev, scores, best
+        self.stats = None
 
 
 def _need(fn, desc, what):
@@ -141,9 +142,24 @@
         for k in range(3):
             g.out[k] = outs[k].data_ptr() if outs[k] is not None else None
         g.workspace, g.workspace_bytes = base + offs[i], int(job.need)
+    sarr = None
+    if any(job.stats for job in jobs):
+        sarr = (_lib.GroupStats * len(jobs))()
+        for i, job in enumerate(jobs):
+            st = job.stats or {}
+            s_ = sarr[i]
+            s_.max_a = st["max_a"].data_ptr() if st.get("max_a") is not None else None
+            s_.max_b = st["max_b"].data_ptr() if st.get("max_b") is not None else None
+            mass = st.get("row_mass")
+            s_.row_mass = mass.data_ptr() if mass is not None else None
+            s_.mass_rows, s_.mass_cols = (mass.numel(), int(st["mass_cols"])) if mass is not None else (0, 0)
+            keep.append(st)
     with torch.cuda.device(dev):
         ev = C.c_void_p(inputs_ready.cuda_event) if inputs_ready is not None else C.c_void_p(0)
-        rc = lib.p4v_calibrate_group(arr, len(jobs), stream_ptr(dev), ev)
+        if sarr is None:
+            rc = lib.p4v_calibrate_group(arr, len(jobs), stream_ptr(dev), ev)
+        else:
+            rc = lib.p4v_calibrate_group_stats(arr, sarr, len(jobs), stream_ptr(dev), ev)
     _lib.check(rc, "p4v_calibrate_group")
     del keep
     return jobs
@@ -549,6 +565,32 @@
     _lib.check(rc, "p4v_multi_copy")
 
 
+def capture_append(table, n, index, max_bytes, dev):
+    lib = _lib.load()
+    with torch.cuda.device(dev):
+        rc = lib.p4v_capture_append(ptr(table), int(n), int(index), int(max_bytes), stream_ptr(dev))
+    _lib.check(rc, "p4v_capture_append")
+
+
+def append_row(src, dst, kind=_lib.APPEND_NONE, stat=None, a=0, b=0):
+    return [src.data_ptr(), dst.data_ptr(), src.numel() * 4, int(kind), stat.data_ptr() if stat is not None else 0, int(a), int(b), 0]
+
+
+def debug_row_mass(grad2d):
+    assert grad2d.is_cuda and grad2d.dtype == torch.float32 and grad2d.dim() == 2 and grad2d.is_contiguous()
+    out = torch.empty(grad2d.shape[0], dtype=torch.float32, device=grad2d.device)
+    with torch.cuda.device(grad2d.device):
+        rc = _lib.load().p4v_debug_row_mass(ptr(grad2d), grad2d.shape[0], grad2d.shape[1], ptr(out), stream_ptr(grad2d.device))
+    _lib.check(rc, "p4v_debug_row_mass")
+    return out
+
+
+def stats_skipped(reset=False):
+    out = (C.c_int64 * 2)()
+    _lib.check(_lib.load().p4v_debug_stats_skipped(out, int(bool(reset))), "p4v_debug_stats_skipped")
+    return {"absmax": int(out[0]), "row_mass": int(out[1])}
+
+
 def stats_enable(flag):
     _lib.load().p4v_stats_enable(int(bool(flag)))
 
diff --git a/ptq4vit_amd/utils/quant_calib.py b/ptq4vit_amd/utils/quant_calib.py
--- a/ptq4vit_amd/utils/quant_calib.py
+++ b/ptq4vit_amd/utils/quant_calib.py
@@ -119,6 +119,61 @@
         return False
     span = 1 + sum((t.shape[k] - 1) * t.stride(k) for k in range(t.dim()))
     return span == t.numel() and t.stride(0) == max(t.stride())
+
+
+def _head_chunk(t):
+    if t.dim() != 4 or min(t.shape) < 1:
+        return None
+    _b, h, r, c = t.shape
+    chunk = r * c
+    if chunk < 4 or t.stride(0) != h * chunk or t.stride(1) != chunk:
+        return None
+    if (t.stride(2), t.stride(3)) not in ((c, 1), (1, r)):
+        return None
+    return chunk
+
+
+def _capture_stat_plan(m, tensors, with_grad):
+    from .. import _lib
+    plan = [(None, _lib.APPEND_NONE, 0, 0)] * len(tensors)
+    big = 1 << 31
+    if isinstance(m, MinMaxQuantMatMul):
+        for k, role in ((0, "max_a"), (1, "max_b")):
+            t = tensors[k]
+            chunk = _head_chunk(t)
+            if chunk is not None and t.shape[1] <= _lib.APPEND_MAX_UNITS and t.numel() < big:
+                plan[k] = (role, _lib.APPEND_ABSMAX, chunk, int(t.shape[1]))
+    elif isinstance(m, MinMaxQuantLinear):
+        if getattr(m, "n_a", 1) == 1 and tensors[0].numel() < big:
+            plan[0] = ("max_a", _lib.APPEND_MAX if getattr(m, "_postgelu", False) else _lib.APPEND_ABSMAX, 0, 1)
+    elif isinstance(m, MinMaxQuantConv2d):
+        if tensors[0].numel() < big:
+            plan[0] = ("max_a", _lib.APPEND_ABSMAX, 0, 1)
+    if with_grad and getattr(m, "metric", None) == "hessian" and isinstance(m, (MinMaxQuantMatMul, MinMaxQuantLinear)):
+        g = tensors[-1]
+        if g.dim() >= 2 and g.is_contiguous() and g.shape[-1] >= 1 and g.numel() > 0:
+            plan[-1] = ("row_mass", _lib.APPEND_ROW_MASS, int(g.shape[-1]), g.numel() // int(g.shape[-1]))
+    return plan
+
+
+def _stats_match_job(st, job):
+    from .. import _lib
+    d, ins = job.desc, job.inputs
+    if job.kind == _lib.JOB_MATMUL:
+        acts, grad = (ins[0], ins[1]), ins[3]
+        ok = all(st.get(r) is None or st[r].numel() == d.heads for r in ("max_a", "max_b"))
+    else:
+        acts, grad = (ins[2], None), ins[4]
+        ok = st.get("max_b") is None
+        if job.kind == _lib.JOB_LINEAR and st.get("max_a") is not None:
+            ok = ok and d.n_a == 1 and bool(d.twin_postgelu) == bool(st["signed"])
+    for r, t in zip(("max_a", "max_b"), acts):
+        if st.get(r) is not None:
+            ok = ok and t is not None and t.data_ptr() == st["ptr"][r]
+    if st.get("row_mass") is not None:
+        ok = ok and grad is not None and grad.data_ptr() == st["ptr"]["row_mass"] and d.metric == _lib.METRICS["hessian"] \
+            and grad.numel() == st["row_mass"].numel() * st["mass_cols"]
+    return bool(ok)
 
 
 def _groupable(m):
@@ -457,7 +512,8 @@
         n_lanes = max(1, min(want, n_sub, len(lanes)))
         t_ = tick(f"graphs ready ({len(lanes)} instance(s))", t_)
         from .. import engine
-        flat_dsts, plans = [], []
+        flat_dsts, plans, lane_plans = [], [], []
+        from .. import _lib
         key_names = tuple(names)
         recipe0 = lanes[0].setdefault("recipes", {}).get(key_names)
         if recipe0 is None:
@@ -470,6 +526,14 @@
                     is_block.append(_same_dense_block(c, t))
                     del c
             recipe0 = lanes[0]["recipes"][key_names] = {"n_sub": n_sub, "layout": layout, "is_block": is_block}
+        want_stats = os.environ.get("P4V_CAPTURE_STATS", "1") != "0"
+        stat_sig = tuple((getattr(m, "n_a", 1), getattr(m, "metric", None), getattr(m, "_postgelu", False))
+                         for m in (self.wrapped_modules[n] for n in names)) if want_stats else None
+        if want_stats and stat_sig not in recipe0.setdefault("stat_plans", {}):
+            sp = []
+            for n in names:
+                sp += _capture_stat_plan(self.wrapped_modules[n], *lanes[0]["statics"][n])
+            recipe0["stat_plans"][stat_sig] = sp
         if recipe0["n_sub"] != n_sub:
             lanes[0]["recipes"].pop(key_names)
             return self._capture_passes_graph(names, dev, bs, raw_pred_softmax)
@@ -490,6 +554,8 @@
             if hasattr(m, "metric"):
                 d_["raw_grad"] = full[-1] if with_g else None
             flat_dsts += full
+        no_stat = (None, 0, 0, 0)
+        stat_plan = list(recipe0["stat_plans"][stat_sig]) if want_stats else [no_stat] * len(flat_dsts)
         for li in range(n_lanes):
             statics = lanes[li]["statics"]
             srcs = []
@@ -499,14 +565,56 @@
             if lane_blocks is None:
                 lane_blocks = [bool(b) and _same_dense_block(d, t) for d, t, b in zip(flat_dsts, srcs, recipe0["is_block"])]
                 lanes[li]["is_block"][key_names] = lane_blocks
-            block = [(d, t) for d, t, b in zip(flat_dsts, srcs, lane_blocks) if b]
+            if want_stats:
+                lane_sp = lanes[li].setdefault("stat_plans", {}).get((key_names, stat_sig))
+                if lane_sp is None:
+                    lane_sp = []
+                    for n in names:
+                        lane_sp += _capture_stat_plan(self.wrapped_modules[n], *statics[n])
+                    lanes[li]["stat_plans"][(key_names, stat_sig)] = lane_sp
+                stat_plan = [p_ if b and p_ == q_ else no_stat for p_, q_, b in zip(stat_plan, lane_sp, lane_blocks)]
+            lane_plans.append((lanes[li], srcs, lane_blocks))
+        offs, n_words = [], 0
+        for role, _kind, _a, b_ in stat_plan:
+            offs.append(n_words)
+            n_words += 0 if role is None else b_ * n_sub if role == "row_mass" else b_
+        arena = torch.zeros(n_words, dtype=torch.int32, device=dev) if n_words else None
+        stat_views = [None] * len(stat_plan)
+        k_ = 0
+        for n in names:
+            m = self.wrapped_modules[n]
+            st = {"ptr": {}}
+            for _t in lanes[0]["statics"][n][0]:
+                role, kind, a_, b_ = stat_plan[k_]
+                if role is not None:
+                    v = arena[offs[k_]:offs[k_] + (b_ * n_sub if role == "row_mass" else b_)]
+                    stat_views[k_] = st[role] = v.view(torch.float32) if role == "row_mass" else v
+                    st["ptr"][role] = flat_dsts[k_].data_ptr()
+                    if role == "row_mass":
+                        st["mass_cols"] = a_
+                    elif role == "max_a":
+                        st["signed"] = kind == _lib.APPEND_MAX
+                k_ += 1
+            m.__dict__.pop("_p4v_capture_stats", None)
+            if st["ptr"]:
+                m.__dict__["_p4v_capture_stats"] = st
+        for lane, srcs, lane_blocks in lane_plans:
             other = [(d, t) for d, t, b in zip(flat_dsts, srcs, lane_blocks) if not b]
-            table, max_bytes = None, 0
-            if block:
-                rows = [[t.data_ptr(), d.data_ptr(), t.numel() * 4] for d, t in block]
+            table, max_bytes, rows = None, 0, []
+            for d, t, b, v, (_role, kind, a_, b_) in zip(flat_dsts, srcs, lane_blocks, stat_views, stat_plan):
+                if b:
+                    rows.append(engine.append_row(t, d, kind, v, a_, b_) if arena is not None else [t.data_ptr(), d.data_ptr(), t.numel() * 4])
+            if rows:
                 table = torch.tensor(rows, dtype=torch.int64).to(dev, non_blocking=True)
                 max_bytes = max(r[2] for r in rows)
-            plans.append((lanes[li], table, len(block), max_bytes, other))
+            plans.append((lane, table, len(rows), max_bytes, other))
+        if trace:
+            cnt, gib = {"max": 0, "row mass": 0, "plain": 0, "torch copy": 0}, {"max": 0.0, "row mass": 0.0, "plain": 0.0, "torch copy": 0.0}
+            for d, b, p_ in zip(flat_dsts, lane_plans[0][2], stat_plan):
+                what = "torch copy" if not b else "plain" if p_[0] is None else "row mass" if p_[0] == "row_mass" else "max"
+                cnt[what] += 1
+                gib[what] += d.numel() * 4 / 2**30
+            print("[capture] append: " + ", ".join(f"{cnt[k]} {k} ({gib[k]:.2f} GiB)" for k in cnt), file=sys.stderr, flush=True)
         t_ = tick(f"caches allocated ({sum(d.numel() * 4 for d in flat_dsts) / 2**30:.1f} GiB)", t_)
         main = torch.cuda.current_stream(dev)
         streams = [main] if n_lanes == 1 else engine.side_streams(dev, n_lanes)
@@ -521,7 +629,10 @@
                 entry["tgt"].copy_(raw_pred_softmax[st:st + bs])
                 entry["graph"].replay()
                 if table is not None:
-                    engine.multi_copy(table, n_block, i, max_bytes, dev)
+                    if arena is not None:
+                        engine.capture_append(table, n_block, i, max_bytes, dev)
+                    else:
+                        engine.multi_copy(table, n_block, i, max_bytes, dev)
                     if i < n_lanes:
                         table.record_stream(streams[i % n_lanes])
                 for d, t in other:
@@ -685,6 +796,9 @@
                             if batch and acc + held > budget:
                                 break
                             todo.pop(0)
+                            st = m.__dict__.pop("_p4v_capture_stats", None)
+                            if st is not None and _stats_match_job(st, job):
+                                job.stats = st
                             batch.append(n); jobs.append(job); acc += held
                         if not batch:
                             continue
@@ -860,6 +974,8 @@
                     self._search_grouped(grp, calls, inputs_ready=cap_done)
                 else:
                     self._search_concurrent(grp, n_streams)
+                for n in grp:
+                    self.wrapped_modules[n].__dict__.pop("_p4v_capture_stats", None)
                 if cap_done is not None:
                     ref = torch.cuda.Event(enable_timing=True)
                     ref.record(torch.cuda.current_stream(_dev_of(self.net)))
```

After: 645.0. 3.0% lower.
